# uguryagmur/RealTimeObjectDetection

Hardware: AMD Instinct MI355X
Metric: frames/sec YOLOv3 608x608 bs=8 (Darknet.forward + write_results; 2 batches in flight, write_results_async on a second stream) (higher is better)
Workload: dtype f16x2-split (3 MFMA products, f32 accumulate); 1 GPU; YOLOv3 cfg 608x608 batch=8 per GPU, split-f16 MFMA conv + fused head + GPU NMS (BASELINE configs[2]); precision=f16s3, tiles=autotune (this run), parallelism=frame-shard x1, in_flight_batches=2, detections_last_step=1699, candidates_last_step=1914, f16_range_overflow=False

## Files before the change

### realtimeobjectdetection_amd/csrc/capi.cpp

```cpp
#include <cstring>
#include <new>

#include "plan.h"

namespace rtod { const std::string& last_error_string(); }
using namespace rtod;

struct rtod_plan { Plan p; };

#define RTOD_GUARD_BEGIN try {
#define RTOD_GUARD_END                                                                   \
    } catch (const std::bad_alloc&) { set_error("out of host memory"); return RTOD_E_ARG; } \
      catch (const std::exception& e) { set_error("internal error: %s", e.what()); return RTOD_E_ARG; } \
      catch (...) { set_error("internal error"); return RTOD_E_ARG; }

extern "C" {

int rtod_version(void) { return 100; }

int rtod_last_error(char* buf, size_t len) {
    if (!buf || !len) return RTOD_E_ARG;
    const std::string& e = last_error_string();
    const size_t n = e.size() < len - 1 ? e.size() : len - 1;
    memcpy(buf, e.data(), n);
    buf[n] = 0;
    return RTOD_OK;
}

int rtod_device_count(int* out) {
    if (!out) return RTOD_E_ARG;
    int n = 0;
    hipError_t e = hipGetDeviceCount(&n);
    if (e != hipSuccess) { *out = 0; (void)hipGetLastError(); return RTOD_OK; }
    *out = n;
    return RTOD_OK;
}

static int plan_create(const char* cfg_text, size_t len, int height, int width, int max_batch, int device, rtod_plan** out) {
    rtod_plan* h = new rtod_plan();
    h->p.height = height; h->p.width = width; h->p.max_batch = max_batch; h->p.device = device;
    int rc = h->p.parse(std::string(cfg_text, len));
    if (!rc) rc = h->p.resolve_shapes();
    if (!rc) rc = h->p.plan_buffers();
    if (rc) { delete h; return rc; }
    *out = h;
    return RTOD_OK;
}

int rtod_plan_create(const char* cfg_text, size_t len, int height, int width, int max_batch, int device, rtod_plan** out) {
    RTOD_GUARD_BEGIN
    if (!cfg_text || !out) { set_error("plan_create: null pointer"); return RTOD_E_ARG; }
    *out = nullptr;
    if (height < 1 || width < 1 || max_batch < 1 || device < 0) { set_error("plan_create: bad geometry %dx%d batch %d device %d", height, width, max_batch, device); return RTOD_E_ARG; }
    if (height != width) { set_error("plan_create: only square inputs are supported (the reference derives every stride from net_info['height']); use rtod_plan_create_rect"); return RTOD_E_ARG; }
    return plan_create(cfg_text, len, height, width, max_batch, device, out);
    RTOD_GUARD_END
}

int rtod_plan_create_rect(const char* cfg_text, size_t len, int height, int width, int max_batch, int device, rtod_plan** out) {
    RTOD_GUARD_BEGIN
    if (!cfg_text || !out) { set_error("plan_create_rect: null pointer"); return RTOD_E_ARG; }
    *out = nullptr;
    if (height < 1 || width < 1 || max_batch < 1 || device < 0) { set_error("plan_create_rect: bad geometry %dx%d batch %d device %d", height, width, max_batch, device); return RTOD_E_ARG; }
    return plan_create(cfg_text, len, height, width, max_batch, device, out);
    RTOD_GUARD_END
}

int rtod_plan_destroy(rtod_plan* plan) {
    delete plan;
    return RTOD_OK;
}

int rtod_plan_get_info(const rtod_plan* plan, rtod_plan_info* o) {
    if (!plan || !o) { set_error("plan_get_info: null pointer"); return RTOD_E_ARG; }
    const Plan& p = plan->p;
    memset(o, 0, sizeof(*o));
    o->n_layers = (int32_t)p.layers.size(); o->n_launches = (int32_t)p.launches.size();
    o->height = p.height; o->width = p.width; o->max_batch = p.max_batch;
    o->total_rows = p.total_rows; o->attrs = p.attrs;
    o->n_weight_floats = p.n_weight_floats; o->conv_flops_per_frame = p.conv_flops;
    o->arena_bytes = p.arena_floats * 4; o->packed_weight_bytes = p.packed_floats * 4;
    return RTOD_OK;
}

int rtod_plan_get_launch(const rtod_plan* plan, int index, rtod_launch_info* out) {
    if (!plan || !out || index < 0 || index >= (int)plan->p.launches.size()) { set_error("plan_get_launch: bad index"); return RTOD_E_ARG; }
    plan->p.fill_launch_info(index, out, plan->p.tuned.empty() ? plan->p.max_batch : plan->p.tuned.rbegin()->first);
    return RTOD_OK;
}

int rtod_plan_describe(const rtod_plan* plan, char* buf, size_t len, size_t* needed) {
    RTOD_GUARD_BEGIN
    if (!plan) { set_error("plan_describe: null plan"); return RTOD_E_ARG; }
    const std::string s = plan->p.describe();
    if (needed) *needed = s.size() + 1;
    if (buf && len) {
        const size_t n = s.size() < len - 1 ? s.size() : len - 1;
        memcpy(buf, s.data(), n);
        buf[n] = 0;
    }
    return RTOD_OK;
    RTOD_GUARD_END
}

const char* rtod_conv_variant_name(int variant) {
    if (variant == 100 + STEM2_VARIANT) return "conv_stem2_f16s3<2 x 4x16, stem + 3x3 s2 + 1x1>";
    if (variant >= 100 + PATCH_VARIANT_BASE && variant < 100 + PATCH_VARIANT_BASE + PATCH_MODES) return conv_patch_mode_info(variant - 100 - PATCH_VARIANT_BASE).name;
    if (variant >= 100 + PWD_VARIANT_BASE && variant < 100 + PWD_VARIANT_BASE + PWD_MODES) return conv_pwd_mode_info(variant - 100 - PWD_VARIANT_BASE).name;
    if (variant >= 100 + RING_VARIANT_BASE && variant < 100 + RING_VARIANT_BASE + RING_MODES) return conv_ring_mode_info(variant - 100 - RING_VARIANT_BASE).name;
    if (variant >= 100 + BAND_VARIANT_BASE && variant < 100 + BAND_VARIANT_BASE + BAND_MODES) return conv_band_mode_info(variant - 100 - BAND_VARIANT_BASE).name;
    if (variant >= 100 && variant < 100 + HV_COUNT) return conv_f16s3_variant_info(variant - 100).name;
    if (variant < 0 || variant % 10 >= CV_COUNT || variant / 10 > 2) return "";
    static const char* const kSliced[2][CV_COUNT] = {
        {"conv_igemm_f32<128x128,w64x64,k-slices>", "conv_igemm_f32<128x64,w64x32,k-slices>", "conv_igemm_f32<64x64,w32x32,k-slices>", "conv_igemm_f32<128x32,w32x32,k-slices>"},
        {"conv_igemm_f32<128x128,w64x64,wg per k-slice>", "conv_igemm_f32<128x64,w64x32,wg per k-slice>", "conv_igemm_f32<64x64,w32x32,wg per k-slice>", "conv_igemm_f32<128x32,w32x32,wg per k-slice>"}};
    if (variant >= 10) return kSliced[variant / 10 - 1][variant % 10];
    return conv_variant_info(variant).name;
}

int rtod_conv_kernel_name(int variant, int epilogue, char* buf, size_t len) {
    if (!buf || len == 0) { set_error("conv_kernel_name: null buffer"); return RTOD_E_ARG; }
    int n = -1;
    if (variant >= 100 + PATCH_VARIANT_BASE) n = conv_patch_kernel_name(variant - 100 - PATCH_VARIANT_BASE, epilogue, buf, len);
    else if (variant >= 100 + PWD_VARIANT_BASE) n = conv_pwd_kernel_name(variant - 100 - PWD_VARIANT_BASE, epilogue, buf, len);
    else if (variant >= 100 + RING_VARIANT_BASE) n = conv_ring_kernel_name(variant - 100 - RING_VARIANT_BASE, epilogue, buf, len);
    else if (variant >= 100 + BAND_VARIANT_BASE) n = conv_band_kernel_name(variant - 100 - BAND_VARIANT_BASE, epilogue, buf, len);
    else if (variant >= 100) n = conv_f16s3_kernel_name(variant - 100, epilogue, buf, len);
    else n = conv_f32_kernel_name(variant, buf, len);
    if (n < 0 || (size_t)n >= len) { set_error("conv_kernel_name: unknown variant %d or buffer too small", variant); return RTOD_E_ARG; }
    return RTOD_OK;
}

int rtod_plan_launch_kernel_name(const rtod_plan* plan, int index, char* buf, size_t len) {
    RTOD_GUARD_BEGIN
    if (!plan || !buf || len == 0 || index < 0 || index >= (int)plan->p.launches.size()) { set_error("launch_kernel_name: bad args"); return RTOD_E_ARG; }
    rtod_launch_info li;
    plan->p.fill_launch_info(index, &li, plan->p.tuned.empty() ? plan->p.max_batch : plan->p.tuned.rbegin()->first);
    buf[0] = 0;
    if (li.kind != LK_CONV || li.flops_per_frame == 0) return RTOD_OK;
    int epi = li.fused_decode ? 2 : (li.fused_pointwise ? (li.fused_residual ? 4 : 3) : (li.fused_residual ? 1 : 0));
    if (plan->p.precision == 2 && li.variant >= 100) epi |= EPI_F16;
    int n = -1;
    if (li.variant == 100 + STEM2_VARIANT) n = conv_stem2_kernel_name(li.fused_pointwise, buf, len);
    else return rtod_conv_kernel_name(li.variant, epi, buf, len);
    if (n < 0 || (size_t)n >= len) { set_error("launch_kernel_name: buffer too small"); return RTOD_E_ARG; }
    return RTOD_OK;
    RTOD_GUARD_END
}

int rtod_plan_set_precision(rtod_plan* plan, int mode) {
    if (!plan || mode < 0 || mode > 2) { set_error("set_precision: mode must be 0 (fp32), 1 (f16 split) or 2 (plain f16)"); return RTOD_E_ARG; }
    if (plan->p.d_weights) { set_error("set_precision: must be called before rtod_plan_load_weights"); return RTOD_E_STATE; }
    if (mode >= 1) { const int rc = plan->p.check_split_supported(mode); if (rc) return rc; }
    plan->p.precision = mode;
    plan->p.layout_weights();
    return RTOD_OK;
}

int rtod_plan_set_option(rtod_plan* plan, const char* name, int value) {
    RTOD_GUARD_BEGIN
    if (!plan) { set_error("set_option: null plan"); return RTOD_E_ARG; }
    return plan->p.set_option(name, value);
    RTOD_GUARD_END
}

int rtod_plan_set_overflow_flag(rtod_plan* plan, int32_t* flag_dev) {
    if (!plan) { set_error("set_overflow_flag: null plan"); return RTOD_E_ARG; }
    plan->p.overflow_flag = flag_dev;
    return RTOD_OK;
}

int rtod_plan_load_weights(rtod_plan* plan, const float* w, size_t n_floats) {
    RTOD_GUARD_BEGIN
    if (!plan) { set_error("load_weights: null plan"); return RTOD_E_ARG; }
    return plan->p.load_weights(w, n_floats);
    RTOD_GUARD_END
}

int rtod_forward(rtod_plan* plan, const float* x_dev, int batch, float* out_dev, void* stream) {
    RTOD_GUARD_BEGIN
    if (!plan) { set_error("forward: null plan"); return RTOD_E_ARG; }
    return plan->p.forward(x_dev, batch, out_dev, (hipStream_t)stream, nullptr);
    RTOD_GUARD_END
}

int rtod_plan_autotune(rtod_plan* plan, const float* x_dev, int batch, float* out_dev, void* stream) {
    RTOD_GUARD_BEGIN
    if (!plan) { set_error("autotune: null plan"); return RTOD_E_ARG; }
    return plan->p.forward(x_dev, batch, out_dev, (hipStream_t)stream, nullptr, true);
    RTOD_GUARD_END
}

int rtod_plan_get_tiles(const rtod_plan* plan, int batch, int* variants, int capacity) {
    if (!plan) { set_error("get_tiles: null plan"); return RTOD_E_ARG; }
    auto it = plan->p.tuned.find(batch);
    if (it == plan->p.tuned.end()) { set_error("get_tiles: batch %d has no tile table (run rtod_plan_autotune first)", batch); return RTOD_E_STATE; }
    const int n = (int)it->second.size();
    if (variants) {
        if (capacity < n) { set_error("get_tiles: capacity %d < %d launches", capacity, n); return RTOD_E_ARG; }
        for (int i = 0; i < n; ++i) variants[i] = it->second[i];
    }
    return n;
}

int rtod_plan_set_tiles(rtod_plan* plan, int batch, const int* variants, int count) {
    RTOD_GUARD_BEGIN
    if (!plan) { set_error("set_tiles: null plan"); return RTOD_E_ARG; }
    return plan->p.set_tiles(batch, variants, count);
    RTOD_GUARD_END
}

int rtod_forward_timed(rtod_plan* plan, const float* x_dev, int batch, float* out_dev, void* stream, float* launch_ms) {
    RTOD_GUARD_BEGIN
    if (!plan || !launch_ms) { set_error("forward_timed: null pointer"); return RTOD_E_ARG; }
    return plan->p.forward(x_dev, batch, out_dev, (hipStream_t)stream, launch_ms);
    RTOD_GUARD_END
}

int rtod_plan_set_train_decode(rtod_plan* plan, int train) {
    if (!plan) { set_error("set_train_decode: null plan"); return RTOD_E_ARG; }
    plan->p.train_decode = train ? 1 : 0;
    return RTOD_OK;
}

int rtod_plan_set_keep_all_layers(rtod_plan* plan, int keep) {
    if (!plan) { set_error("set_keep_all_layers: null plan"); return RTOD_E_ARG; }
    if (plan->p.d_arena) { set_error("set_keep_all_layers: must be called before rtod_plan_load_weights"); return RTOD_E_STATE; }
    plan->p.keep_all = keep != 0;
    plan->p.assign_arena();
    return RTOD_OK;
}

int rtod_plan_layer_shape(const rtod_plan* plan, int layer, int* c, int* h, int* w) {
    if (!plan || layer < 0 || layer >= (int)plan->p.layers.size() || !c || !h || !w) { set_error("layer_shape: bad args"); return RTOD_E_ARG; }
    const View v = plan->p.view_of(layer);
    if (v.C == 0) { set_error("layer %d is fused into its consumer and has no materialised output", layer); return RTOD_E_STATE; }
    *c = v.C; *h = v.H; *w = v.W;
    return RTOD_OK;
}

int rtod_plan_read_layer(rtod_plan* plan, int layer, int batch, float* out_dev_nchw, void* stream) {
    RTOD_GUARD_BEGIN
    if (!plan || layer < 0 || layer >= (int)plan->p.layers.size()) { set_error("read_layer: bad args"); return RTOD_E_ARG; }
    if (batch < 1 || batch > plan->p.max_batch) { set_error("read_layer: bad batch"); return RTOD_E_ARG; }
    const View v = plan->p.view_of(layer);
    if (!v.base) { set_error("layer %d has no materialised output (fused) or weights not loaded", layer); return RTOD_E_STATE; }
    return launch_view_to_nchw(v, batch, out_dev_nchw, (hipStream_t)stream);
    RTOD_GUARD_END
}

int rtod_plan_bn_batch_stats(rtod_plan* plan, int layer, double* mean_host, double* var_host, int channels, void* stream) {
    RTOD_GUARD_BEGIN
    if (!plan || !mean_host || !var_host || layer < 0 || layer >= (int)plan->p.layers.size()) { set_error("bn_batch_stats: bad args"); return RTOD_E_ARG; }
    if (!plan->p.opt_bn_batch_stats || !plan->p.d_bn_stats) { set_error("bn_batch_stats: the plan does not run batch-statistics BatchNorm (option bn_batch_stats, weights loaded)"); return RTOD_E_STATE; }
    for (const auto& pc : plan->p.convs) {
        if (pc.layer != layer) continue;
        if (pc.stats_off < 0 || channels != plan->p.layers[layer].cout) { set_error("bn_batch_stats: layer %d has no BatchNorm / %d channels", layer, plan->p.layers[layer].cout); return RTOD_E_ARG; }
        RTOD_HIP(hipSetDevice(plan->p.device));
        RTOD_HIP(hipStreamSynchronize((hipStream_t)stream));
        RTOD_HIP(hipMemcpy(mean_host, plan->p.d_bn_stats + pc.stats_off, sizeof(double) * channels, hipMemcpyDeviceToHost));
        RTOD_HIP(hipMemcpy(var_host, plan->p.d_bn_stats + pc.stats_off + pc.Npad, sizeof(double) * channels, hipMemcpyDeviceToHost));
        return RTOD_OK;
    }
    set_error("bn_batch_stats: layer %d is not a convolution", layer);
    return RTOD_E_ARG;
    RTOD_GUARD_END
}

int rtod_plan_bn_update_running(rtod_plan* plan, int batch, float* const* running_mean_dev, float* const* running_var_dev, int n_bn,
                                double momentum, void* stream) {
    RTOD_GUARD_BEGIN
    if (!plan || !running_mean_dev || !running_var_dev || batch < 1 || batch > plan->p.max_batch) { set_error("bn_update_running: bad args"); return RTOD_E_ARG; }
    if (!plan->p.opt_bn_batch_stats || !plan->p.d_bn_stats) { set_error("bn_update_running: the plan does not run batch-statistics BatchNorm (option bn_batch_stats, weights loaded)"); return RTOD_E_STATE; }
    std::vector<BnUpdateEntry> ent;
    for (const auto& pc : plan->p.convs) {
        if (pc.stats_off < 0) continue;
        const int k = (int)ent.size();
        if (k >= n_bn) { set_error("bn_update_running: %d pointers for more BatchNorm layers", n_bn); return RTOD_E_ARG; }
        if (!running_mean_dev[k] || !running_var_dev[k]) { set_error("bn_update_running: null buffer %d", k); return RTOD_E_ARG; }
        const View v = plan->p.view_of(pc.layer);
        const auto& L = plan->p.layers[pc.layer];
        const int64_t n = (int64_t)batch * L.hout * L.wout;
        (void)v;
        ent.push_back(BnUpdateEntry{running_mean_dev[k], running_var_dev[k], pc.stats_off, (double)n / (double)(n > 1 ? n - 1 : 1), pc.Npad, L.cout});
    }
    if ((int)ent.size() != n_bn) { set_error("bn_update_running: the plan has %d BatchNorm layers, %d pointers given", (int)ent.size(), n_bn); return RTOD_E_ARG; }
    if (ent.empty()) return RTOD_OK;
    RTOD_HIP(hipSetDevice(plan->p.device));
    return launch_bn_update_running(ent.data(), (int)ent.size(), plan->p.d_bn_stats, momentum, (hipStream_t)stream);
    RTOD_GUARD_END
}

int rtod_predict_transform(const float* raw_dev, int batch, int attrs, int grid, int n_anchors, const float* anchors_wh,
                           int inp_dim, int train, float* out_dev, void* stream) {
    RTOD_GUARD_BEGIN
    if (!raw_dev || !out_dev || !anchors_wh) { set_error("predict_transform: null pointer"); return RTOD_E_ARG; }
    if (batch < 1 || attrs < 5 || grid < 1 || n_anchors < 1 || n_anchors > 4 || inp_dim < grid) { set_error("predict_transform: bad shape"); return RTOD_E_ARG; }
    const int stride = inp_dim / grid;
    if (inp_dim / stride != grid) { set_error("predict_transform: grid %d inconsistent with inp_dim %d (util.py:195 would mis-shape)", grid, inp_dim); return RTOD_E_ARG; }
    DecodeArgs d; d.enabled = 1; d.GH = grid; d.GW = grid; d.attrs = attrs; d.n_anchors = n_anchors; d.train = train ? 1 : 0; d.stride = (float)stride;
    for (int a = 0; a < n_anchors; ++a) {
        d.aw[a] = (float)((double)anchors_wh[2 * a] / (double)stride);
        d.ah[a] = (float)((double)anchors_wh[2 * a + 1] / (double)stride);
    }
    d.img_stride = (int64_t)grid * grid * n_anchors * attrs; d.head_off = 0;
    return launch_decode(raw_dev, (int64_t)n_anchors * attrs * grid * grid, (int64_t)grid * grid, grid, 1, batch, d, out_dev, (hipStream_t)stream);
    RTOD_GUARD_END
}

int rtod_confidence_mask(const float* pred_dev, int64_t rows, int attrs, float confidence, float* out_dev, void* stream) {
    return launch_confidence_mask(pred_dev, rows, attrs, confidence, out_dev, (hipStream_t)stream);
}

int rtod_bbox_iou(const float* box1_dev, const float* boxes_dev, int k, int row_stride, float* iou_dev, void* stream) {
    return launch_bbox_iou(box1_dev, boxes_dev, k, row_stride, iou_dev, (hipStream_t)stream);
}

int rtod_prep_image(const uint8_t* img_dev, int height, int width, int bgr, int inp_dim, float* out_dev, void* stream) {
    RTOD_GUARD_BEGIN
    return launch_prep_image(img_dev, height, width, bgr, inp_dim, out_dev, (hipStream_t)stream);
    RTOD_GUARD_END
}

int rtod_prep_frames(const uint8_t* frames_dev, int batch, int height, int width, int bgr, int out_h, int out_w, float* out_dev, void* stream) {
    RTOD_GUARD_BEGIN
    return launch_prep_frames(frames_dev, batch, height, width, bgr, out_h, out_w, out_dev, (hipStream_t)stream);
    RTOD_GUARD_END
}

int rtod_write_results_workspace(int batch, int n, size_t* bytes) {
    if (!bytes || batch < 1 || n < 1) { set_error("write_results_workspace: bad args"); return RTOD_E_ARG; }
    *bytes = nms_workspace_bytes(batch, n);
    return RTOD_OK;
}

int rtod_write_results(const float* pred_dev, int batch, int n, int num_class, float confidence, float nms_conf,
                       float* out_dev, int cap, int32_t* counts_dev, void* workspace_dev, size_t workspace_bytes, void* stream) {
    RTOD_GUARD_BEGIN
    return launch_write_results(pred_dev, batch, n, num_class, confidence, nms_conf, out_dev, cap, counts_dev,
                                workspace_dev, workspace_bytes, (hipStream_t)stream);
    RTOD_GUARD_END
}

int rtod_nms_class_offset(const float* pred_dev, int batch, int n, int num_class, float confidence, float iou_thr, float max_wh, int max_det,
                          float* out_dev, int cap, int32_t* counts_dev, void* workspace_dev, size_t workspace_bytes, void* stream) {
    RTOD_GUARD_BEGIN
    return launch_nms_class_offset(pred_dev, batch, n, num_class, confidence, iou_thr, max_wh, max_det, out_dev, cap, counts_dev,
                                   workspace_dev, workspace_bytes, (hipStream_t)stream);
    RTOD_GUARD_END
}

}
```

### realtimeobjectdetection_amd/csrc/conv_bandd_common.h

```cpp
#pragma once
#include "conv_f16s3_common.h"

namespace rtod {

#ifdef RTOD_TIMELINE
constexpr int BD_EPI_BLOCKS = 2048;
static __device__ unsigned long long g_bandd_epi[BD_EPI_BLOCKS * 5];
#define BD_ESTAMP(slot) { const unsigned long long tn_ = __builtin_amdgcn_s_memtime(); et_[slot] += tn_ - eprev_; eprev_ = tn_; }
#else
#define BD_ESTAMP(slot)
#endif

template <int NBASE, int PER = 2> __device__ __forceinline__ void bandd_wait_vmcnt_plus(int n) {
    static_assert(((NBASE == 4 || NBASE == 8) && PER == 2) || ((NBASE == 2 || NBASE == 4) && PER == 1), "two B sets of 1, 2 or 4 loads");
    asm volatile("" : "+s"(n));
    if (n == 0) vmcnt<NBASE>();
    else if (n == 1) vmcnt<NBASE + PER>();
    else if (n == 2) vmcnt<NBASE + 2 * PER>();
    else if (n == 3) vmcnt<NBASE + 3 * PER>();
    else if (n == 4) vmcnt<NBASE + 4 * PER>();
    else vmcnt<NBASE + 5 * PER>();
}

template <int BM, int BN, int WM, int WN, int NT, int RG, bool RES, int KG, bool F16 = false>
__device__ __forceinline__ void bandd_epilogue(const ConvArgs& a, f32x4 (&acc)[WM / 16][WN / 16], unsigned char* smem, int bm, int bn, int tid,
                                               int wm, int wn, int lr, int lh, int M, int kg) {
    constexpr int TM = WM / 16, TN = WN / 16, MT = 16, NE = 4, TS = BN;
    static_assert(BM % RG == 0 && RG % 16 == 0, "epilogue pass");
#ifdef RTOD_TIMELINE
    unsigned long long et_[5] = {0, 0, 0, 0, 0};
    unsigned long long eprev_ = __builtin_amdgcn_s_memtime();
#endif
    float* T = reinterpret_cast<float*>(smem);
    float amax = 0.f;
    const float escale = SPLIT_SCALE;
    constexpr int GPR = BN / 8;
    constexpr int NG = (RG * GPR + NT - 1) / NT;
    constexpr int NP = BM / RG;
    float bias_j[TN], inv_j[TN];
#pragma unroll
    for (int j = 0; j < TN; ++j) {
        const int n = bn * BN + wn * WN + j * MT + lr;
        const int nc = n < a.Cout ? n : 0;
        const float b = a.bias[nc], iv = a.inv_scale[nc];
        bias_j[j] = n < a.Cout ? b : 0.f; inv_j[j] = n < a.Cout ? iv : 0.f;
    }
    f16x8 rq_h[RES ? NP : 1][RES ? NG : 1], rq_l[RES ? NP : 1][RES ? NG : 1];
    static_assert(NT % GPR == 0, "epilogue items: constant row step");
    constexpr int RSTEP = NT / GPR;
    const int er = tid / GPR, ec8 = (tid - er * GPR) * 8;
    const bool ecol = bn * BN + ec8 < a.Cout;
    if constexpr (RES) {
        const _Float16* rh0 = reinterpret_cast<const _Float16*>(a.res) + a.res_coff + bn * BN;
        const int64_t rstep = (int64_t)RSTEP * 2 * a.res_ldc;
        const _Float16* const q0 = rh0 + (int64_t)(bm * BM + er) * 2 * a.res_ldc + ec8;
#pragma unroll
        for (int p = 0; p < NP; ++p) {
            const _Float16* q = q0 + (int64_t)(p * RG) * 2 * a.res_ldc;
#pragma unroll
            for (int i = 0; i < NG; ++i) {
                const int m = bm * BM + p * RG + er + i * RSTEP;
                const _Float16* qq = (er + i * RSTEP < RG && m < M && ecol) ? q : rh0;
                rq_h[p][i] = *reinterpret_cast<const f16x8*>(qq);
                if constexpr (!F16) rq_l[p][i] = *reinterpret_cast<const f16x8*>(qq + a.res_ldc);
                q += rstep;
            }
        }
    }
    __syncthreads();
    BD_ESTAMP(0)
#pragma unroll
    for (int rg = 0; rg < BM; rg += RG) {
        if constexpr (KG == 2) {
            if (kg == 1) {
#pragma unroll
                for (int i = 0; i < TM; ++i) {
                    const int r0 = wm * WM + i * MT;
                    if (r0 >= rg && r0 < rg + RG) {
#pragma unroll
                        for (int j = 0; j < TN; ++j)
#pragma unroll
                            for (int e = 0; e < NE; ++e) T[(r0 - rg + e + 4 * lh) * TS + wn * WN + j * MT + lr] = acc[i][j][e];
                    }
                }
            }
            __syncthreads();
        }
        if (KG == 1 || kg == 0) {
#pragma unroll
            for (int j = 0; j < TN; ++j) {
                const int nl = wn * WN + j * MT + lr;
                const float bias = bias_j[j] * escale, inv = inv_j[j] * escale;
                auto col = [&](auto act) {
#pragma unroll
                    for (int i = 0; i < TM; ++i) {
                        const int r0 = wm * WM + i * MT;
                        if (r0 >= rg && r0 < rg + RG) {
#pragma unroll
                            for (int e = 0; e < NE; ++e) {
                                const int rl = r0 - rg + e + 4 * lh;
                                float s = acc[i][j][e];
                                if constexpr (KG == 2) s += T[rl * TS + nl];
                                float v = s * inv + bias;
                                if constexpr (decltype(act)::value == 2) v = silu_scaled(v, 1.0f / escale);
                                else if constexpr (decltype(act)::value == 1) v = __builtin_fmaxf(v, v * 0.1f);
                                T[rl * TS + nl] = v;
                            }
                        }
                    }
                };
                if (a.leaky == 2) col(std::integral_constant<int, 2>{});
                else if (a.leaky) col(std::integral_constant<int, 1>{});
                else col(std::integral_constant<int, 0>{});
            }
        }
        BD_ESTAMP(1)
        __syncthreads();
        BD_ESTAMP(2)
        _Float16* oq = reinterpret_cast<_Float16*>(a.out) + a.out_coff + bn * BN + (int64_t)(bm * BM + rg + er) * 2 * a.out_ldc + ec8;
        const int64_t ostep = (int64_t)RSTEP * 2 * a.out_ldc;
#pragma unroll
        for (int gi = 0; gi < NG; ++gi, oq += ostep) {
            const int r = er + gi * RSTEP;
            const int m = bm * BM + rg + r;
            if (r >= RG || m >= M || !ecol) continue;
            const f32x4 v0 = *reinterpret_cast<const f32x4*>(T + r * TS + ec8);
            const f32x4 v1 = *reinterpret_cast<const f32x4*>(T + r * TS + ec8 + 4);
            float v[8] = {v0[0], v0[1], v0[2], v0[3], v1[0], v1[1], v1[2], v1[3]};
            if constexpr (RES && F16) {
                const f16x8 qh = rq_h[rg / RG][gi];
#pragma unroll
                for (int e = 0; e < 8; ++e) v[e] += (float)qh[e];
            } else if constexpr (RES) {
                const f16x8 qh = rq_h[rg / RG][gi], ql = rq_l[rg / RG][gi];
#pragma unroll
                for (int e = 0; e < 8; ++e) v[e] += (float)qh[e] + (float)ql[e];
            }
            if constexpr (F16) {
                f16x8 ph;
#pragma unroll
                for (int e = 0; e < 8; ++e) ph[e] = f16_sat(v[e], amax);
                store_act16(oq, ph, false);
            } else {
                f16x8 ph, pl;
#pragma unroll
                for (int e = 0; e < 8; ++e) { _Float16 h, l; split_f16(v[e], h, l, amax); ph[e] = h; pl[e] = l; }
                store_act16(oq, ph, false);
                store_act16(oq + a.out_ldc, pl, false);
            }
        }
        BD_ESTAMP(3)
        if (rg + RG < BM) __syncthreads();
        BD_ESTAMP(4)
    }
#ifdef RTOD_TIMELINE
    if (threadIdx.x == 0 && blockIdx.x < BD_EPI_BLOCKS) for (int i = 0; i < 5; ++i) g_bandd_epi[blockIdx.x * 5 + i] = et_[i];
#endif
    split_overflow_report(a.ovf, amax);
}

}
```

### realtimeobjectdetection_amd/csrc/conv_pwd_f16s3.hip

```cpp
#include "conv_bandd_common.h"

namespace rtod {

template <int BM, int NW, int NST, int MINW, int EPI>
__global__ __launch_bounds__(NW * 64, MINW)
void conv_pwd_f16s3_kernel(const ConvArgs a, const int grid_m, const int grid_n) {
    constexpr bool F16 = epi_f16(EPI);
    constexpr int LB = F16 ? 2 : 4, LP = F16 ? 1 : 2;
    constexpr int BN = NW * 32, NT = NW * 64, TM = BM / 16, TN = 2;
    constexpr int SLAB = BM * 256;
    constexpr int NP = BM / 8;
    constexpr int NPP = (NP + NW - 1) / NW;
    static_assert(BM % 16 == 0 && NPP >= 1 && NPP <= 8, "slab pieces per wave");
    static_assert(NST >= 2 && NST <= 4, "ring depth");
    constexpr int RG = BM * BN * 4 <= 32768 ? BM : (BM / 2) * BN * 4 <= 32768 ? BM / 2 : BM / 4;
    constexpr int WAIT_B = 2 * LB + LP * NPP;
    constexpr int WAIT_SLAB = 2 * LB + (NST - 2) * (LP * NPP + 2 * LB);
    constexpr int WAIT_SLAB_PRO = 2 * LB + (NST - 2) * LP * NPP;

    extern __shared__ __attribute__((aligned(16))) unsigned char smem[];
    const int nwg = grid_m * grid_n;
    int bid = blockIdx.x;
    if (!a.xcd_by_n) bid = xcd_remap(bid, nwg);
    const int bm = bid / grid_n, bn = bid - bm * grid_n;
    const int tid = (int)threadIdx.x;
    const int wave = __builtin_amdgcn_readfirstlane(tid >> 6), lane = tid & 63;
    const int lr = lane & 15, lh = lane >> 4;
    const int M = a.B * a.Hi * a.Wi;
    const int m0 = bm * BM;
    const unsigned PS = (unsigned)a.in_ldc * 4u;
    const unsigned lo_plane = (unsigned)a.in_ldc * 2u;

    const __amdgpu_buffer_rsrc_t rs_a = buffer_rsrc(a.in, a.in_bytes);
    const __amdgpu_buffer_rsrc_t rs_wh = buffer_rsrc(a.w_hi, a.w_bytes);
    const __amdgpu_buffer_rsrc_t rs_wl = buffer_rsrc(a.w_lo, a.w_bytes);
    const unsigned lds0 = (unsigned)(size_t)smem;
    const int NS = a.Cin / 64;

    unsigned dma_vo[NPP];
#pragma unroll
    for (int k = 0; k < NPP; ++k) {
        const int p = wave + k * NW;
        const int r = lane >> 3;
        const int m = m0 + p * 8 + r;
        dma_vo[k] = (p < NP && m < M) ? (unsigned)m * PS + (unsigned)(a.in_coff + (((lane & 7) ^ r) << 3)) * 2u : OOB;
    }
    auto dma_slab = [&](int js) __attribute__((always_inline)) {
        const bool live = js < NS;
        const unsigned soff = (unsigned)js * 128u;
        const unsigned base = lds0 + (unsigned)((js % NST) * SLAB);
#pragma unroll
        for (int k = 0; k < NPP; ++k) {
            const int p = wave + k * NW;
            const unsigned dst = p < NP ? base + (unsigned)((p >> 1) * 4096 + (p & 1) * 1024) : lds0 + (unsigned)(NST * SLAB);
            if constexpr (F16) lds_dma(rs_a, live ? dma_vo[k] : OOB, soff, dst);
            else lds_dma_pair<0x800>(rs_a, live ? dma_vo[k] : OOB, soff, lo_plane + soff, dst);
        }
    };
    const int wn = wave;
    const int n0 = bn * BN + wn * 32;
    const unsigned bvoff = n0 + lr < a.Npad ? (unsigned)((n0 + lr) * 32 + lh * 8) * 2u : OOB;
    const unsigned wchunk = (unsigned)a.Npad * (HBK * 2);
    const int nsteps = 2 * NS;
    u32x4 Bq[4][TN][2];
    auto load_b = [&](int t, u32x4 (&q)[TN][2]) __attribute__((always_inline)) {
        const unsigned vo = t < nsteps ? bvoff : OOB;
        const unsigned koff = (unsigned)t * wchunk;
        q[0][0] = buffer_load_b128(rs_wh, vo, koff);
        if constexpr (!F16) q[0][1] = buffer_load_b128(rs_wl, vo, koff);
        q[1][0] = buffer_load_b128<1024>(rs_wh, vo, koff);
        if constexpr (!F16) q[1][1] = buffer_load_b128<1024>(rs_wl, vo, koff);
    };

    f32x4 acc[TM][TN];
#pragma unroll
    for (int i = 0; i < TM; ++i)
#pragma unroll
        for (int j = 0; j < TN; ++j)
#pragma unroll
            for (int e = 0; e < 4; ++e) acc[i][j][e] = 0.f;

    typedef const f16x8 __attribute__((address_space(3))) lds_f16x8;
    const int rbase = (lr >> 3) * 1024 + (lr & 7) * 128;
    int xq0 = rbase + ((lh ^ (lr & 7)) << 4);
    int xq1 = rbase + (((4 + lh) ^ (lr & 7)) << 4);
    f16x8 Ah[3], Al[3];
    auto read_unit = [&](int q, int i, int slotoff, f16x8& h, f16x8& l) __attribute__((always_inline)) {
        const int o = (q ? xq1 : xq0) + slotoff;
        h = *reinterpret_cast<lds_f16x8*>((unsigned)(o + 4096 * i));
        if constexpr (!F16) l = *reinterpret_cast<lds_f16x8*>((unsigned)(o + 4096 * i + 2048));
    };

#pragma unroll
    for (int s = 0; s < NST - 1; ++s) dma_slab(s);
    load_b(0, Bq[0]);
    load_b(1, Bq[1]);

    __builtin_amdgcn_s_setprio(2);
    auto slab_body = [&](int j, auto par_c) __attribute__((always_inline)) {
        constexpr int par = decltype(par_c)::value;
        asm volatile("" : "+v"(xq0), "+v"(xq1));
        if (j < NST - 1) vmcnt<WAIT_SLAB_PRO>(); else vmcnt<WAIT_SLAB>();
        __builtin_amdgcn_sched_barrier(0);
        __builtin_amdgcn_s_barrier();
        dma_slab(j + NST - 1);
        const int slotoff = (int)lds0 + (j % NST) * SLAB;
        read_unit(0, 0, slotoff, Ah[0], Al[0]);
        read_unit(1 / TM, 1 % TM, slotoff, Ah[1], Al[1]);
        __builtin_amdgcn_sched_barrier(0);
#pragma unroll
        for (int u = 0; u < 2 * TM; ++u) {
            const int q = u / TM, i = u % TM;
            if (i == 0) {
                if (q == 0) load_b(2 * j + 2, Bq[(2 * par + 2) % 4]); else load_b(2 * j + 3, Bq[(2 * par + 3) % 4]);
                vmcnt<WAIT_B>();
                if (q == 0) tie_bset<F16>(Bq[2 * par]); else tie_bset<F16>(Bq[2 * par + 1]);
                __builtin_amdgcn_sched_barrier(0);
            }
            if (u + 2 < 2 * TM) read_unit((u + 2) / TM, (u + 2) % TM, slotoff, Ah[(u + 2) % 3], Al[(u + 2) % 3]);
            const f16x8 ah = Ah[u % 3], al = Al[u % 3];
#pragma unroll
            for (int jn = 0; jn < TN; ++jn) {
                const f16x8 bh = __builtin_bit_cast(f16x8, Bq[2 * par + q][jn][0]);
                if constexpr (F16) { acc[i][jn] = __builtin_amdgcn_mfma_f32_16x16x32_f16(ah, bh, acc[i][jn], 0, 0, 0); continue; }
                const f16x8 bl = __builtin_bit_cast(f16x8, Bq[2 * par + q][jn][1]);
                acc[i][jn] = __builtin_amdgcn_mfma_f32_16x16x32_f16(al, bh, acc[i][jn], 0, 0, 0);
                acc[i][jn] = __builtin_amdgcn_mfma_f32_16x16x32_f16(ah, bl, acc[i][jn], 0, 0, 0);
                acc[i][jn] = __builtin_amdgcn_mfma_f32_16x16x32_f16(ah, bh, acc[i][jn], 0, 0, 0);
            }
            __builtin_amdgcn_sched_barrier(0);
        }
    };
#pragma unroll 1
    for (int j = 0; j < NS; j += 2) {
        slab_body(j, std::integral_constant<int, 0>{});
        if (j + 1 < NS) slab_body(j + 1, std::integral_constant<int, 1>{});
    }
    vmcnt<0>();
    tie_bset<F16>(Bq[0]); tie_bset<F16>(Bq[1]); tie_bset<F16>(Bq[2]); tie_bset<F16>(Bq[3]);
    __builtin_amdgcn_sched_barrier(0);
    __builtin_amdgcn_s_setprio(0);

    bandd_epilogue<BM, BN, BM, 32, NT, RG, epi_kind(EPI) == EPI_SPLIT_RES, 1, F16>(a, acc, smem, bm, bn, tid, 0, wn, lr, lh, M, 0);
}

template <int BM, int NW, int NST, int MINW>
static int launch_pwd(const ConvArgs& a, hipStream_t s) {
    constexpr int BN = NW * 32, NT = NW * 64;
    constexpr int RG = BM * BN * 4 <= 32768 ? BM : (BM / 2) * BN * 4 <= 32768 ? BM / 2 : BM / 4;
    const int M = a.B * a.Ho * a.Wo;
    const int gm = (M + BM - 1) / BM, gn = (a.Cout + BN - 1) / BN;
    ConvArgs ax = a;
    ax.xcd_by_n = (gn % 8 == 0 && (int64_t)a.Cout * a.K > (int64_t)M * a.Cin) ? 1 : 0;
    constexpr int ring_bytes = NST * BM * 256 + ((BM / 8) % NW ? 4096 : 0), epi_bytes = RG * BN * 4;
    constexpr int lds = ring_bytes > epi_bytes ? ring_bytes : epi_bytes;
    static_assert(lds <= 160 * 1024, "LDS");
    const int fe = a.f16 ? 1 : 0;
    auto k_res = fe ? conv_pwd_f16s3_kernel<BM, NW, NST, MINW, EPI_SPLIT_RES | EPI_F16> : conv_pwd_f16s3_kernel<BM, NW, NST, MINW, EPI_SPLIT_RES>;
    auto k_plain = fe ? conv_pwd_f16s3_kernel<BM, NW, NST, MINW, EPI_SPLIT | EPI_F16> : conv_pwd_f16s3_kernel<BM, NW, NST, MINW, EPI_SPLIT>;
    if constexpr (lds > 64 * 1024) {
        static std::atomic<unsigned long long> attr_done[2] = {{0}, {0}};
        if (int rc = lds_opt_in(attr_done[fe], lds, "conv_pwd_f16s3", k_res, k_plain)) return rc;
    }
    if (a.res) hipLaunchKernelGGL(k_res, dim3(gm * gn), dim3(NT), lds, s, ax, gm, gn);
    else hipLaunchKernelGGL(k_plain, dim3(gm * gn), dim3(NT), lds, s, ax, gm, gn);
    return hip_fail(hipGetLastError(), "conv_pwd_f16s3 launch");
}

#define RTOD_PWD_TILES(X) \
    X(0, 64, 4, 3, 3) X(1, 32, 4, 3, 3) X(2, 128, 4, 3, 1) X(3, 64, 8, 3, 1) X(4, 64, 4, 2, 3) X(5, 32, 4, 4, 3) X(6, 96, 4, 2, 3) X(7, 96, 4, 3, 2) X(8, 48, 4, 3, 3) X(9, 48, 4, 4, 3) X(10, 64, 2, 2, 4)

#define RTOD_X_INFO(idx, bm, nw, nst, minw) {bm, nw * 32, "conv_pwd_f16s3<" #bm "x" #nw "w,r" #nst ">"},
static const ConvVariantInfo kPwdModes[PWD_MODES] = { RTOD_PWD_TILES(RTOD_X_INFO) };
#undef RTOD_X_INFO
const ConvVariantInfo& conv_pwd_mode_info(int idx) { return kPwdModes[idx < 0 || idx >= PWD_MODES ? 0 : idx]; }

bool conv_pwd_supported(int ksize, int stride, int pad, int cin) { return ksize == 1 && stride == 1 && pad == 0 && cin >= 64 && cin % 64 == 0; }

int conv_pwd_kernel_name(int idx, int epi, char* buf, size_t len) {
#define RTOD_X_NAME(i, bm, nw, nst, minw) \
    if (idx == i) return snprintf(buf, len, "void rtod::conv_pwd_f16s3_kernel<" #bm ", " #nw ", " #nst ", " #minw ", %d>(rtod::ConvArgs, int, int)", epi);
    RTOD_PWD_TILES(RTOD_X_NAME)
#undef RTOD_X_NAME
    return -1;
}

int launch_conv_pwd_f16s3(const ConvArgs& a, int idx, hipStream_t s) {
    if (int rc = check_split_conv_args(a, "launch_conv_pwd", true)) return rc;
    if (!conv_pwd_supported(a.kh, a.stride, a.pad, a.Cin) || a.kw != 1 || a.Ho != a.Hi || a.Wo != a.Wi || a.dec.enabled || a.pw_wh) {
        set_error("launch_conv_pwd: unsupported shape (k=%d s=%d pad=%d Cin=%d)", a.kh, a.stride, a.pad, a.Cin); return RTOD_E_ARG;
    }
    if (a.in_ldc % 8 || a.in_coff % 8 || a.K != a.Kpad || a.K != a.Cin || a.Npad % 128) { set_error("launch_conv_pwd: bad view / K"); return RTOD_E_ARG; }
    switch (idx) {
#define RTOD_X_CASE(i, bm, nw, nst, minw) case i: return launch_pwd<bm, nw, nst, minw>(a, s);
        RTOD_PWD_TILES(RTOD_X_CASE)
#undef RTOD_X_CASE
    }
    set_error("launch_conv_pwd: mode %d unsupported", idx);
    return RTOD_E_ARG;
}

}
```

### realtimeobjectdetection_amd/csrc/plan.cpp

```cpp
#include "plan.h"

#include <algorithm>
#include <cctype>
#include <cmath>
#include <cstdarg>
#include <cstdlib>
#include <cstring>
#include <map>
#include <mutex>
#include <sstream>

namespace rtod {

static thread_local std::string g_err;

void set_error(const char* fmt, ...) {
    char buf[1024];
    va_list ap;
    va_start(ap, fmt);
    vsnprintf(buf, sizeof(buf), fmt, ap);
    va_end(ap);
    g_err = buf;
}
const std::string& last_error_string() { return g_err; }

int hip_fail(hipError_t e, const char* what) {
    if (e == hipSuccess) return RTOD_OK;
    set_error("HIP error %d (%s) at %s", (int)e, hipGetErrorString(e), what);
    return RTOD_E_HIP;
}

const char* layer_type_name(int t) {
    static const char* n[] = {"convolutional", "shortcut", "route", "upsample", "maxpool", "yolo"};
    return (t >= 0 && t < 6) ? n[t] : "?";
}

Plan::~Plan() {
    for (auto e : events) (void)hipEventDestroy(e);
    if (d_arena) (void)hipFree(d_arena);
    if (d_scratch) (void)hipFree(d_scratch);
    if (d_bn_stats) (void)hipFree(d_bn_stats);
    if (d_bn_partial) (void)hipFree(d_bn_partial);
    if (d_weights) (void)hipFree(d_weights);
}

static std::string rstrip(const std::string& s) {
    size_t e = s.size();
    while (e > 0 && isspace((unsigned char)s[e - 1])) --e;
    return s.substr(0, e);
}
static std::string lstrip(const std::string& s) {
    size_t b = 0;
    while (b < s.size() && isspace((unsigned char)s[b])) ++b;
    return s.substr(b);
}

static bool to_int(const std::string& s, int& out) {
    const std::string t = rstrip(lstrip(s));
    if (t.empty()) return false;
    char* end = nullptr;
    long v = strtol(t.c_str(), &end, 10);
    if (*end) return false;
    out = (int)v;
    return true;
}

static std::vector<std::string> split(const std::string& s, char d) {
    std::vector<std::string> out;
    std::string cur;
    for (char c : s) {
        if (c == d) { out.push_back(cur); cur.clear(); } else cur.push_back(c);
    }
    out.push_back(cur);
    return out;
}

struct Block { std::string type; std::map<std::string, std::string> kv; };

static int parse_blocks(const std::string& text, std::vector<Block>& blocks) {
    Block cur;
    bool have = false;
    for (const std::string& raw : split(text, '\n')) {
        if (raw.empty()) continue;
        if (raw[0] == '#') continue;
        const std::string line = rstrip(lstrip(raw));
        if (line.empty()) continue;
        if (line[0] == '[') {
            if (have) blocks.push_back(cur);
            cur = Block();
            have = true;
            cur.type = rstrip(line.substr(1, line.size() >= 2 ? line.size() - 2 : 0));
        } else {
            const auto parts = split(line, '=');
            if (parts.size() != 2 || !have) { set_error("cfg: malformed line '%s'", line.c_str()); return RTOD_E_CFG; }
            cur.kv[rstrip(parts[0])] = lstrip(parts[1]);
        }
    }
    if (have) blocks.push_back(cur);
    if (blocks.empty() || blocks[0].type != "net") { set_error("cfg: first block must be [net]"); return RTOD_E_CFG; }
    return RTOD_OK;
}

#define CFG_INT(blk, key, var)                                                                  \
    do {                                                                                        \
        auto _it = (blk).kv.find(key);                                                          \
        if (_it == (blk).kv.end() || !to_int(_it->second, var)) {                               \
            set_error("cfg: layer %d [%s]: missing/invalid '%s'", i, (blk).type.c_str(), key);  \
            return RTOD_E_CFG;                                                                  \
        }                                                                                       \
    } while (0)

int Plan::parse(const std::string& text) {
    std::vector<Block> blocks;
    int rc = parse_blocks(text, blocks);
    if (rc) return rc;
    net_info = blocks[0].kv;
    layers.clear();
    for (size_t bi = 1; bi < blocks.size(); ++bi) {
        const Block& b = blocks[bi];
        const int i = (int)bi - 1;
        Layer L;
        L.index = i;
        if (b.type == "convolutional") {
            L.type = LT_CONV;
            int bn = 0;
            auto it = b.kv.find("batch_normalize");
            L.bn = (it != b.kv.end() && to_int(it->second, bn) && bn != 0);
            int padflag = 0;
            CFG_INT(b, "filters", L.cout);
            CFG_INT(b, "size", L.size);
            CFG_INT(b, "stride", L.stride);
            CFG_INT(b, "pad", padflag);
            L.pad = padflag ? (L.size - 1) / 2 : 0;
            auto act = b.kv.find("activation");
            if (act == b.kv.end()) { set_error("cfg: layer %d: missing activation", i); return RTOD_E_CFG; }
            L.leaky = act->second == "leaky";
            L.act = L.leaky ? 1 : (act->second == "silu" || act->second == "swish") ? 2 : 0;
            if (L.cout < 1 || L.size < 1 || L.stride < 1) { set_error("cfg: layer %d: bad conv geometry", i); return RTOD_E_CFG; }
        } else if (b.type == "upsample") {
            L.type = LT_UPSAMPLE;
            int st = 0;
            CFG_INT(b, "stride", st);
            L.stride = 2;
            auto md = b.kv.find("mode");
            L.nearest = md != b.kv.end() && md->second == "nearest";
        } else if (b.type == "maxpool") {
            L.type = LT_MAXPOOL;
            CFG_INT(b, "size", L.size);
            CFG_INT(b, "stride", L.stride);
            int sym = 0;
            auto sy = b.kv.find("symmetric");
            if (sy != b.kv.end() && to_int(sy->second, sym) && sym) L.pool_pad = (L.size - 1) / 2;
            if (L.size < 1 || L.stride < 1) { set_error("cfg: layer %d: bad pool geometry", i); return RTOD_E_CFG; }
        } else if (b.type == "shortcut") {
            L.type = LT_SHORTCUT;
            int from = 0;
            CFG_INT(b, "from", from);
            L.srcs = {i - 1, i + from};
        } else if (b.type == "route") {
            L.type = LT_ROUTE;
            auto it = b.kv.find("layers");
            if (it == b.kv.end()) { set_error("cfg: layer %d: route without layers", i); return RTOD_E_CFG; }
            for (const std::string& tok : split(it->second, ',')) {
                int v = 0;
                if (!to_int(tok, v)) { set_error("cfg: layer %d: bad route entry '%s'", i, tok.c_str()); return RTOD_E_CFG; }
                L.srcs.push_back(v > 0 ? v : i + v);
            }
            if (L.srcs.empty() || L.srcs.size() > 4) {
                set_error("cfg: layer %d: route with %zu sources unsupported", i, L.srcs.size()); return RTOD_E_CFG;
            }
        } else if (b.type == "yolo") {
            L.type = LT_YOLO;
            auto m = b.kv.find("mask"), a = b.kv.find("anchors");
            if (m == b.kv.end() || a == b.kv.end()) { set_error("cfg: layer %d: yolo without mask/anchors", i); return RTOD_E_CFG; }
            std::vector<int> av;
            for (const std::string& tok : split(a->second, ',')) { int v; if (!to_int(tok, v)) { set_error("cfg: bad anchor"); return RTOD_E_CFG; } av.push_back(v); }
            for (const std::string& tok : split(m->second, ',')) {
                int v;
                if (!to_int(tok, v) || v < 0 || 2 * v + 1 >= (int)av.size()) { set_error("cfg: layer %d: bad mask", i); return RTOD_E_CFG; }
                L.anchors.push_back({av[2 * v], av[2 * v + 1]});
            }
            CFG_INT(b, "classes", L.classes);
            auto dv = b.kv.find("decode");
            L.decode_v5 = dv != b.kv.end() && dv->second == "v5";
            if (L.anchors.empty() || L.anchors.size() > 4) { set_error("cfg: layer %d: 1..4 anchors per head supported", i); return RTOD_E_CFG; }
        } else {
            set_error("Unknown block error: A unknown block is provided: [%s]", b.type.c_str());
            return RTOD_E_CFG;
        }
        layers.push_back(L);
    }
    if (layers.empty()) { set_error("cfg: no layers"); return RTOD_E_CFG; }
    return RTOD_OK;
}

int Plan::resolve_shapes() {
    int pc = 3, ph = height, pw = width;
    int row_off = 0;
    int64_t woff = 0;
    conv_flops = 0;
    attrs = 0;
    bool prev_is_decoded = false;
    for (auto& L : layers) {
        const int i = L.index;
        auto src_ok = [&](int s) { return s >= 0 && s < i; };
        if ((L.type == LT_CONV || L.type == LT_UPSAMPLE || L.type == LT_MAXPOOL || L.type == LT_YOLO) && prev_is_decoded) {
            set_error("cfg: layer %d consumes a decoded yolo tensor (unsupported)", i); return RTOD_E_CFG;
        }
        L.cin = pc; L.hin = ph; L.win = pw;
        switch (L.type) {
            case LT_CONV:
                L.hout = (ph + 2 * L.pad - L.size) / L.stride + 1;
                L.wout = (pw + 2 * L.pad - L.size) / L.stride + 1;
                if (L.hout < 1 || L.wout < 1) { set_error("cfg: layer %d: empty conv output", i); return RTOD_E_CFG; }
                L.w_off = woff;
                woff += (L.bn ? 4 : 1) * (int64_t)L.cout + (int64_t)L.cout * L.cin * L.size * L.size;
                conv_flops += 2ll * L.hout * L.wout * L.cout * L.cin * L.size * L.size;
                break;
            case LT_UPSAMPLE: L.cout = pc; L.hout = 2 * ph; L.wout = 2 * pw; break;
            case LT_MAXPOOL:
                L.cout = pc;
                if (L.pool_pad) { L.hout = (ph + 2 * L.pool_pad - L.size) / L.stride + 1; L.wout = (pw + 2 * L.pool_pad - L.size) / L.stride + 1; }
                else if (L.stride != 1) { L.hout = (ph - L.size) / L.stride + 1; L.wout = (pw - L.size) / L.stride + 1; }
                else { L.hout = ph; L.wout = pw; }
                if (L.hout < 1 || L.wout < 1) { set_error("cfg: layer %d: empty pool output", i); return RTOD_E_CFG; }
                break;
            case LT_SHORTCUT: {
                if (i < 1 || !src_ok(L.srcs[1])) { set_error("cfg: layer %d: shortcut source out of range", i); return RTOD_E_CFG; }
                const Layer& a = layers[L.srcs[0]]; const Layer& b = layers[L.srcs[1]];
                if (a.cout != b.cout || a.hout != b.hout || a.wout != b.wout) { set_error("cfg: layer %d: shortcut shape mismatch", i); return RTOD_E_CFG; }
                L.cout = a.cout; L.hout = a.hout; L.wout = a.wout;
                break;
            }
            case LT_ROUTE: {
                int c = 0;
                for (int s : L.srcs) {
                    if (!src_ok(s)) { set_error("cfg: layer %d: route source %d out of range", i, s); return RTOD_E_CFG; }
                    if (layers[s].hout != layers[L.srcs[0]].hout || layers[s].wout != layers[L.srcs[0]].wout) { set_error("cfg: layer %d: route spatial mismatch", i); return RTOD_E_CFG; }
                    c += layers[s].cout;
                }
                L.cout = c; L.cin = c; L.hout = layers[L.srcs[0]].hout; L.wout = layers[L.srcs[0]].wout;
                break;
            }
            case LT_YOLO: {
                if (i < 1) { set_error("cfg: yolo as first layer"); return RTOD_E_CFG; }
                const int A = (int)L.anchors.size();
                if (pc != A * (5 + L.classes)) { set_error("cfg: layer %d: head has %d channels, expected %d", i, pc, A * (5 + L.classes)); return RTOD_E_CFG; }
                if (ph > height || pw > width || height / (height / ph) != ph || width / (width / pw) != pw) {
                    set_error("cfg: layer %d: grid %dx%d does not divide input %dx%d", i, ph, pw, height, width); return RTOD_E_CFG;
                }
                if (height / ph != width / pw) {
                    set_error("cfg: layer %d: head grid %dx%d has stride %d along y but %d along x for input %dx%d (one integer stride on both axes is required)",
                              i, ph, pw, height / ph, width / pw, height, width);
                    return RTOD_E_CFG;
                }
                if (attrs && attrs != 5 + L.classes) { set_error("cfg: heads with different class counts"); return RTOD_E_CFG; }
                attrs = 5 + L.classes;
                L.cout = pc; L.hout = ph; L.wout = pw;
                L.row_offset = row_off; L.rows = ph * pw * A;
                row_off += L.rows;
                break;
            }
        }
        if (L.type == LT_YOLO) {
            prev_is_decoded = true;
            pc = layers[i - 1].cout; ph = layers[i - 1].hout; pw = layers[i - 1].wout;
        } else {
            prev_is_decoded = false;
            pc = L.cout; ph = L.hout; pw = L.wout;
        }
        if (L.type == LT_ROUTE || L.type == LT_SHORTCUT) prev_is_decoded = false;
    }
    total_rows = row_off;
    n_weight_floats = woff;
    if (total_rows == 0) { set_error("cfg: no yolo layer (the reference would return [])"); return RTOD_E_CFG; }
    return RTOD_OK;
}

static int resolve_alias(const std::vector<Layer>& layers, int i) {
    while (layers[i].alias_of >= 0) i = layers[i].alias_of;
    return i;
}

void Plan::reset_planning() {
    for (auto& L : layers) { L.fused_into = -1; L.fused_away = false; L.buf = -1; L.coff = 0; L.alias_of = -1; }
    bufs.clear(); launches.clear(); convs.clear(); input_buf = -1;
    tuned.clear(); tune_cache.clear(); tuning.clear();
}

int Plan::set_option(const char* name, int value) {
    if (!name) { set_error("set_option: null name"); return RTOD_E_ARG; }
    if (d_weights) { set_error("set_option: must be called before rtod_plan_load_weights"); return RTOD_E_STATE; }
    const std::string k(name);
    bool* flag = nullptr; int* num = nullptr;
    if (k == "fuse_pointwise") flag = &opt_fuse_pointwise;
    else if (k == "ring_kernel") flag = &opt_ring_kernel;
    else if (k == "pwd_kernel") flag = &opt_pwd_kernel;
    else if (k == "stem2_kernel") flag = &opt_stem2_kernel;
    else if (k == "k_slices") flag = &opt_k_slices;
    else if (k == "bn_batch_stats") {
        if (value && height != width) { set_error("set_option: bn_batch_stats is not supported on a rectangular plan (%dx%d)", height, width); return RTOD_E_ARG; }
        flag = &opt_bn_batch_stats;
    }
    else if (k == "k_slice_workgroups") flag = &opt_k_slice_workgroups;
    else if (k == "patch_kernel") flag = &opt_patch_kernel;
    else if (k == "stem_kernel") flag = &opt_stem_kernel;
    else if (k == "band_kernel") flag = &opt_band_kernel;
    else if (k == "fuse_shortcut") flag = &opt_fuse_shortcut;
    else if (k == "fuse_decode") flag = &opt_fuse_decode;
    else if (k == "zero_copy_concat") flag = &opt_zero_copy_concat;
    else if (k == "force_f16s3_variant") num = &opt_force_f16s3_variant;
    else if (k == "force_f32_variant") num = &opt_force_f32_variant;
    else { set_error("set_option: unknown option '%s'", name); return RTOD_E_ARG; }
    const bool old_flag = flag ? *flag : false; const int old_num = num ? *num : 0;
    if (flag) *flag = value != 0; else *num = value;
    reset_planning();
    int rc = plan_buffers();
    if (!rc && precision >= 1) rc = check_split_supported(precision);
    if (rc) {
        const std::string msg = last_error_string();
        if (flag) *flag = old_flag; else *num = old_num;
        reset_planning();
        (void)plan_buffers();
        set_error("%s", msg.c_str());
    }
    return rc;
}

int Plan::plan_buffers() {
    const int n = (int)layers.size();
    std::vector<std::vector<int>> cons(n);
    for (const auto& L : layers) {
        const int i = L.index;
        switch (L.type) {
            case LT_CONV: case LT_UPSAMPLE: case LT_MAXPOOL: case LT_YOLO: if (i > 0) cons[i - 1].push_back(i); break;
            case LT_SHORTCUT: case LT_ROUTE: for (int s : L.srcs) cons[s].push_back(i); break;
        }
    }
    for (auto& L : layers) {
        if (L.type == LT_ROUTE && L.srcs.size() == 1) L.alias_of = L.srcs[0];
        if (L.type == LT_YOLO) L.alias_of = L.index - 1;
    }
    for (auto& L : layers) {
        const int i = L.index;
        if (i == 0) continue;
        Layer& P = layers[i - 1];
        if (P.type != LT_CONV || P.fused_into >= 0 || cons[i - 1].size() != 1) continue;
        if (L.type == LT_SHORTCUT && L.srcs[1] != i - 1 && opt_fuse_shortcut) { P.fused_into = i; L.fused_away = true; }
        else if (L.type == LT_YOLO && cons[i].empty() && opt_fuse_decode) { P.fused_into = i; L.fused_away = true; }
    }
    auto materialised = [&](const Layer& L) {
        if (L.alias_of >= 0) return false;
        if (L.type == LT_CONV && L.fused_into >= 0) return false;
        if (L.type == LT_ROUTE) return true;
        return true;
    };
    bufs.clear();
    std::vector<int> placed_buf(n, -1), placed_off(n, 0);
    std::vector<std::vector<std::pair<int, int>>> route_copy(n);
    for (auto& L : layers) {
        if (L.type != LT_ROUTE || L.srcs.size() < 2) continue;
        Buffer b; b.C = L.cout; b.H = L.hout; b.W = L.wout;
        const int bid = (int)bufs.size();
        bufs.push_back(b);
        L.buf = bid; L.coff = 0;
        int off = 0;
        for (int s : L.srcs) {
            const int p = resolve_alias(layers, s);
            const Layer& PL = layers[p];
            const bool can = opt_zero_copy_concat && materialised(PL) && PL.type != LT_ROUTE && placed_buf[p] < 0 && off % 4 == 0 && PL.cout % 4 == 0 &&
                             std::count(L.srcs.begin(), L.srcs.end(), s) == 1;
            if (can) { placed_buf[p] = bid; placed_off[p] = off; }
            else route_copy[L.index].push_back({s, off});
            off += layers[s].cout;
        }
    }
    for (auto& L : layers) {
        if (!materialised(L) || L.buf >= 0) continue;
        if (L.type == LT_YOLO) continue;
        if (placed_buf[L.index] >= 0) { L.buf = placed_buf[L.index]; L.coff = placed_off[L.index]; continue; }
        Buffer b; b.C = L.cout; b.H = L.hout; b.W = L.wout;
        if (b.C % 4) { set_error("layer %d: %d channels not a multiple of 4 (unsupported for an intermediate tensor)", L.index, b.C); return RTOD_E_CFG; }
        L.buf = (int)bufs.size(); L.coff = 0;
        bufs.push_back(b);
    }
    {
        Buffer b; b.C = 4; b.H = height; b.W = width;
        input_buf = (int)bufs.size();
        bufs.push_back(b);
    }
    launches.clear();
    convs.clear();
    if (layers[0].type != LT_CONV) { set_error("cfg: first layer must be convolutional"); return RTOD_E_CFG; }
    const bool use_stem = layers[0].size == 3 && layers[0].pad == 1 && layers[0].cin == 3 && layers[0].cout % 32 == 0 &&
                          layers[0].cout <= 64 && layers[0].fused_into < 0 && opt_stem_kernel && !(opt_bn_batch_stats && layers[0].bn);
    if (!use_stem) { Launch l; l.kind = LK_PACK; l.layer = 0; launches.push_back(l); }
    for (auto& L : layers) {
        const int i = L.index;
        Launch l; l.layer = i;
        switch (L.type) {
            case LT_CONV: {
                l.kind = LK_CONV; l.in_layer = i - 1; l.out_layer = i;
                if (L.fused_into >= 0) {
                    const Layer& F = layers[L.fused_into];
                    if (F.type == LT_SHORTCUT) { l.out_layer = F.index; l.in2_layer = F.srcs[1]; }
                    else {
                        l.out_layer = -2;
                        DecodeArgs d; d.enabled = 1; d.GH = F.hout; d.GW = F.wout; d.attrs = 5 + F.classes; d.n_anchors = (int)F.anchors.size();
                        const int stride = height / F.hout;
                        d.stride = (float)stride;
                        for (size_t a = 0; a < F.anchors.size(); ++a) {
                            d.aw[a] = (float)((double)F.anchors[a].first / (double)stride);
                            d.ah[a] = (float)((double)F.anchors[a].second / (double)stride);
                            if (F.decode_v5) { d.aw[a] = (float)F.anchors[a].first; d.ah[a] = (float)F.anchors[a].second; }
                        }
                        d.v5 = F.decode_v5 ? 1 : 0;
                        d.img_stride = (int64_t)total_rows * attrs; d.head_off = (int64_t)F.row_offset * attrs;
                        l.dec = d;
                    }
                }
                PackedConv pc; pc.layer = i; pc.cin_p = (i == 0) ? 4 : L.cin;
                if (i == 0 && use_stem) { pc.stem = true; l.kind = LK_STEM; }
                if (pc.cin_p % 4) { set_error("layer %d: %d input channels not a multiple of 4", i, pc.cin_p); return RTOD_E_CFG; }
                pc.K = L.size * L.size * pc.cin_p; pc.Kpad = (pc.K + 31) / 32 * 32; pc.Npad = (L.cout + 127) / 128 * 128;
                l.conv_slot = (int)convs.size();
                convs.push_back(pc);
                launches.push_back(l);
                break;
            }
            case LT_UPSAMPLE: l.kind = LK_UPSAMPLE; l.in_layer = i - 1; l.out_layer = i; launches.push_back(l); break;
            case LT_MAXPOOL: l.kind = LK_MAXPOOL; l.in_layer = i - 1; l.out_layer = i; launches.push_back(l); break;
            case LT_SHORTCUT:
                if (!L.fused_away) { l.kind = LK_ADD; l.in_layer = L.srcs[0]; l.in2_layer = L.srcs[1]; l.out_layer = i; launches.push_back(l); }
                break;
            case LT_ROUTE:
                for (auto& sc : route_copy[i]) { Launch c; c.kind = LK_COPY; c.layer = i; c.in_layer = sc.first; c.out_buf = L.buf; c.out_coff = sc.second; c.out_layer = i; launches.push_back(c); }
                break;
            case LT_YOLO:
                if (!L.fused_away) {
                    l.kind = LK_DECODE; l.in_layer = i - 1; l.out_layer = -2;
                    DecodeArgs d; d.enabled = 1; d.GH = L.hout; d.GW = L.wout; d.attrs = 5 + L.classes; d.n_anchors = (int)L.anchors.size();
                    const int stride = height / L.hout;
                    d.stride = (float)stride;
                    for (size_t a = 0; a < L.anchors.size(); ++a) {
                        d.aw[a] = (float)((double)L.anchors[a].first / (double)stride);
                        d.ah[a] = (float)((double)L.anchors[a].second / (double)stride);
                        if (L.decode_v5) { d.aw[a] = (float)L.anchors[a].first; d.ah[a] = (float)L.anchors[a].second; }
                    }
                    d.v5 = L.decode_v5 ? 1 : 0;
                    d.img_stride = (int64_t)total_rows * attrs; d.head_off = (int64_t)L.row_offset * attrs;
                    l.dec = d;
                    launches.push_back(l);
                }
                break;
        }
    }
    for (size_t i = 0; i + 1 < launches.size(); ++i) {
        Launch& h = launches[i]; Launch& g = launches[i + 1];
        if (h.kind != LK_CONV || g.kind != LK_CONV || h.out_layer < 0 || g.out_layer < 0 || g.in2_layer >= 0 || h.pw_host >= 0) continue;
        const Layer& H = layers[h.layer]; const Layer& G = layers[g.layer];
        if (g.in_layer != h.out_layer || G.size != 1 || G.stride != 1 || G.pad != 0 || G.cin != H.cout) continue;
        if (H.cout % 32 || H.cout > 64 || (G.cout != 16 && G.cout != 32 && G.cout != 64) || G.fused_into >= 0) continue;
        if (conv_band_supported(H.size, H.stride, H.pad, H.cin, H.win) && H.hout == H.hin) continue;
        h.pw_guest = (int)i + 1; g.pw_host = (int)i;
    }
    stem2_pattern = false;
    if (launches.size() >= 2 && launches[0].kind == LK_STEM && launches[1].kind == LK_CONV && launches[1].layer == 1 && launches[1].in_layer == 0 &&
        launches[1].in2_layer < 0 && launches[1].out_layer == 1 && cons[0].size() == 1 && n > 1) {
        const Layer& L0 = layers[0]; const Layer& L1 = layers[1];
        int pwc = 0;
        if (launches[1].pw_guest >= 0) pwc = layers[launches[launches[1].pw_guest].layer].cout;
        stem2_pattern = L0.bn && L1.bn && L0.act <= 1 && L1.act <= 1 && (launches[1].pw_guest < 0 || layers[launches[launches[1].pw_guest].layer].act <= 1) && conv_stem2_supported(L0.size, L0.stride, L0.pad, L0.cin, L0.cout, L1.size, L1.stride, L1.pad, L1.cout, pwc) &&
                        (pwc == 0 || pwc == 32);
    }
    const int NB = (int)bufs.size();
    for (auto& b : bufs) { b.first = 1 << 30; b.last = -1; }
    auto touch = [&](int buf, int t) { if (buf < 0) return; bufs[buf].first = std::min(bufs[buf].first, t); bufs[buf].last = std::max(bufs[buf].last, t); };
    auto buf_of_layer = [&](int layer) { if (layer < 0) return input_buf; return layers[resolve_alias(layers, layer)].buf; };
    for (const auto& l : launches) {
        const int t = l.layer;
        if (l.kind == LK_PACK) { touch(input_buf, 0); continue; }
        if (l.kind == LK_STEM) { touch(buf_of_layer(l.out_layer), t); continue; }
        touch(buf_of_layer(l.in_layer), t);
        if (l.in2_layer >= 0) touch(buf_of_layer(l.in2_layer), t);
        if (l.kind == LK_COPY) touch(l.out_buf, t);
        else if (l.out_layer >= 0) touch(buf_of_layer(l.out_layer), t);
        if (l.pw_guest >= 0) touch(buf_of_layer(launches[l.pw_guest].out_layer), t);
    }
    for (int b = 0; b < NB; ++b) {
        if (bufs[b].last < 0) { bufs[b].first = bufs[b].last = 0; }
        bufs[b].floats_per_frame = (int64_t)bufs[b].C * bufs[b].H * bufs[b].W;
    }
    assign_arena();
    layout_weights();
    return RTOD_OK;
}

bool Plan::uses_split(const Layer& L, int cin_p) const {
    return precision >= 1 && L.index > 0;
}

int Plan::check_split_supported(int mode) const {
    const char* pn = mode == 2 ? "f16" : "f16s3";
    if (opt_bn_batch_stats) { set_error("precision %s unsupported with bn_batch_stats (batch-statistics BatchNorm runs on the exact-fp32 kernels)", pn); return RTOD_E_CFG; }
    for (const auto& l : launches) {
        if (l.kind == LK_ADD || l.kind == LK_COPY || l.kind == LK_DECODE) {
            set_error("precision %s unsupported for this cfg (layer %d needs a stand-alone %s kernel); use fp32", pn, l.layer,
                      l.kind == LK_ADD ? "add" : l.kind == LK_COPY ? "copy" : "decode");
            return RTOD_E_CFG;
        }
        if (l.kind == LK_CONV && l.layer > 0) {
            const Layer& L = layers[l.layer];
            if (L.cin % 32 || L.cout % 8 * (l.out_layer != -2)) {
                set_error("precision %s unsupported for this cfg (layer %d: Cin=%d Cout=%d); use fp32", pn, l.layer, L.cin, L.cout);
                return RTOD_E_CFG;
            }
        }
    }
    for (const auto& b : bufs) if (b.C % 8 && &b != &bufs[input_buf]) { set_error("precision %s: a buffer has %d channels (not a multiple of 8)", pn, b.C); return RTOD_E_CFG; }
    return RTOD_OK;
}

void Plan::layout_weights() {
    packed_floats = 0;
    bn_stats_doubles = 0;
    for (auto& pc : convs) {
        pc.stats_off = -1;
        if (opt_bn_batch_stats && layers[pc.layer].bn) { pc.stats_off = bn_stats_doubles; bn_stats_doubles += 2 * (int64_t)pc.Npad; }
    }
    for (auto& pc : convs) {
        const Layer& L = layers[pc.layer];
        pc.split = uses_split(L, pc.cin_p);
        const int64_t panel = (int64_t)pc.Npad * pc.Kpad;
        if (pc.stem && precision >= 1) {
            pc.split = true;
            pc.w_off = packed_floats; packed_floats += 16 * (int64_t)L.cout;
            pc.wl_off = packed_floats; packed_floats += 16 * (int64_t)L.cout;
            pc.s_off = packed_floats; packed_floats += L.cout;
        } else if (pc.stem) {
            pc.w_off = packed_floats; packed_floats += 28 * (int64_t)L.cout;
        } else if (pc.split) {
            pc.w_off = packed_floats; packed_floats += panel / 2;
            pc.wl_off = packed_floats; packed_floats += panel / 2;
            pc.s_off = packed_floats; packed_floats += pc.Npad;
            pc.band = conv_band_supported(L.size, L.stride, L.pad, L.cin, L.win) && L.hout == L.hin &&
                      !(L.fused_into >= 0 && layers[L.fused_into].type == LT_YOLO) && opt_band_kernel;
        } else {
            pc.w_off = packed_floats; packed_floats += panel;
            const int nkc = pc.Kpad / 32;
            pc.slice_chunks = (!opt_k_slices || L.hout * L.wout > 2704 || nkc < 8) ? 0 : nkc >= 32 ? 9 : nkc >= 16 ? 4 : 2;
        }
        pc.b_off = packed_floats; packed_floats += pc.Npad;
        if (opt_bn_batch_stats && L.bn) { pc.bn_off = packed_floats; packed_floats += 2 * (int64_t)pc.Npad; }
        packed_floats = (packed_floats + 63) / 64 * 64;
    }
}

void Plan::assign_arena() {
    const int NB = (int)bufs.size();
    std::vector<int> order(NB);
    for (int i = 0; i < NB; ++i) order[i] = i;
    std::sort(order.begin(), order.end(), [&](int a, int b) { return bufs[a].first != bufs[b].first ? bufs[a].first < bufs[b].first : a < b; });
    std::vector<int> done;
    arena_floats = 0;
    for (int id : order) {
        Buffer& B = bufs[id];
        const int64_t size = (B.floats_per_frame * max_batch + 63) / 64 * 64;
        std::vector<std::pair<int64_t, int64_t>> busy;
        for (int o : done) {
            const Buffer& O = bufs[o];
            if (!keep_all && (O.last < B.first || O.first > B.last)) continue;
            busy.push_back({O.offset, O.offset + (O.floats_per_frame * max_batch + 63) / 64 * 64});
        }
        std::sort(busy.begin(), busy.end());
        int64_t off = 0;
        for (auto& iv : busy) { if (off + size <= iv.first) break; off = std::max(off, iv.second); }
        B.offset = off;
        arena_floats = std::max(arena_floats, off + size);
        done.push_back(id);
    }
}

View Plan::view_of(int layer) const {
    View v;
    if (layer < 0) {
        const Buffer& b = bufs[input_buf];
        v.base = d_arena ? d_arena + b.offset : nullptr; v.ldc = 4; v.coff = 0; v.C = 4; v.H = height; v.W = width;
        return v;
    }
    const Layer& L = layers[resolve_alias(layers, layer)];
    if (L.buf < 0) return v;
    const Buffer& b = bufs[L.buf];
    v.split = precision;
    v.base = d_arena ? d_arena + b.offset : nullptr;
    v.ldc = b.C; v.coff = L.coff; v.C = L.cout; v.H = L.hout; v.W = L.wout;
    return v;
}

static uint16_t f32_to_f16_rn(float f) {
    uint32_t x; memcpy(&x, &f, 4);
    const uint32_t sign = (x >> 16) & 0x8000u;
    x &= 0x7FFFFFFFu;
    if (x >= 0x7F800000u) return (uint16_t)(sign | (x > 0x7F800000u ? 0x7E00u : 0x7C00u));
    if (x >= 0x477FF000u) return (uint16_t)(sign | 0x7C00u);
    if (x < 0x33000001u) return (uint16_t)sign;
    int e = (int)(x >> 23) - 127;
    uint32_t m = (x & 0x7FFFFFu) | 0x800000u;
    int shift = (e < -14) ? (13 + (-14 - e)) : 13;
    uint32_t half_m = m >> shift;
    const uint32_t rem = m & ((1u << shift) - 1), halfway = 1u << (shift - 1);
    if (rem > halfway || (rem == halfway && (half_m & 1))) ++half_m;
    uint32_t out;
    if (e < -14) out = half_m;
    else out = ((uint32_t)(e + 15) << 10) + (half_m - 0x400u);
    return (uint16_t)(sign | out);
}
static float f16_to_f32(uint16_t h) {
    const uint32_t sign = (uint32_t)(h & 0x8000u) << 16;
    const int e = (h >> 10) & 0x1F; const uint32_t m = h & 0x3FFu;
    float v;
    if (e == 0) v = std::ldexp((float)m, -24);
    else if (e == 31) v = m ? NAN : INFINITY;
    else v = std::ldexp((float)(m | 0x400u), e - 25);
    uint32_t x; memcpy(&x, &v, 4); x |= sign; memcpy(&v, &x, 4);
    return v;
}

int Plan::load_weights(const float* w, size_t n) {
    if (!w) { set_error("load_weights: null pointer"); return RTOD_E_ARG; }
    if ((int64_t)n < n_weight_floats) {
        set_error("load_weights: stream has %zu floats, network needs %lld", n, (long long)n_weight_floats);
        return RTOD_E_SIZE;
    }
    RTOD_HIP(hipSetDevice(device));
    std::vector<float> packed((size_t)packed_floats, 0.0f);
    for (const auto& pc : convs) {
        const Layer& L = layers[pc.layer];
        const float* p = w + L.w_off;
        const int C = L.cout, cin = L.cin, k = L.size;
        std::vector<double> scale(C, 1.0);
        float* bias = packed.data() + pc.b_off;
        if (L.bn && opt_bn_batch_stats) {
            float* bnp = packed.data() + pc.bn_off;
            for (int o = 0; o < C; ++o) { bias[o] = 0.f; bnp[o] = p[o]; bnp[pc.Npad + o] = p[C + o]; }
            p += 4 * C;
        } else if (L.bn) {
            const float *beta = p, *gamma = p + C, *mean = p + 2 * C, *var = p + 3 * C;
            for (int o = 0; o < C; ++o) {
                const double s = (double)gamma[o] / std::sqrt((double)var[o] + 1e-5);
                scale[o] = s;
                bias[o] = (float)((double)beta[o] - (double)mean[o] * s);
            }
            p += 4 * C;
        } else {
            for (int o = 0; o < C; ++o) bias[o] = p[o];
            p += C;
        }
        if (pc.stem && pc.split) {
            uint16_t* wh = reinterpret_cast<uint16_t*>(packed.data() + pc.w_off);
            uint16_t* wl = reinterpret_cast<uint16_t*>(packed.data() + pc.wl_off);
            float* inv = packed.data() + pc.s_off;
            const int64_t per_o = (int64_t)cin * k * k;
            for (int o = 0; o < C; ++o) {
                double mx = 0.0;
                for (int64_t q = 0; q < per_o; ++q) mx = std::max(mx, std::fabs((double)p[o * per_o + q] * scale[o]));
                int e = 0;
                if (mx > 0.0) { int ex; std::frexp(mx, &ex); e = 13 - ex; }
                e = std::max(-24, std::min(40, e));
                const double ps = std::ldexp(1.0, e);
                inv[o] = (float)(std::ldexp(1.0, -e) / (double)ACT_SCALE_F16S3);
                for (int q = 0; q < 32; ++q) { wh[o * 32 + q] = 0; wl[o * 32 + q] = 0; }
                for (int c = 0; c < cin; ++c)
                    for (int ky = 0; ky < k; ++ky)
                        for (int kx = 0; kx < k; ++kx) {
                            const float v = (float)((double)p[(((int64_t)o * cin + c) * k + ky) * k + kx] * scale[o]);
                            const float vs = (float)((double)v * ps);
                            const uint16_t h = f32_to_f16_rn(vs);
                            const int idx = o * 32 + (ky * k + kx) * 3 + c;
                            wh[idx] = h; wl[idx] = f32_to_f16_rn(vs - f16_to_f32(h));
                        }
            }
        } else if (pc.stem) {
            float* wp = packed.data() + pc.w_off;
            for (int o = 0; o < C; ++o)
                for (int c = 0; c < cin; ++c)
                    for (int ky = 0; ky < k; ++ky)
                        for (int kx = 0; kx < k; ++kx) {
                            const float v = p[(((int64_t)o * cin + c) * k + ky) * k + kx];
                            wp[(int64_t)((ky * k + kx) * 3 + c) * C + o] = (float)((double)v * scale[o]);
                        }
        } else if (!pc.split) {
            float* wp = packed.data() + pc.w_off;
            for (int o = 0; o < C; ++o)
                for (int c = 0; c < cin; ++c)
                    for (int ky = 0; ky < k; ++ky)
                        for (int kx = 0; kx < k; ++kx) {
                            const float v = p[(((int64_t)o * cin + c) * k + ky) * k + kx];
                            wp[(int64_t)o * pc.Kpad + (ky * k + kx) * pc.cin_p + c] = (float)((double)v * scale[o]);
                        }
        } else {
            uint16_t* wh = reinterpret_cast<uint16_t*>(packed.data() + pc.w_off);
            uint16_t* wl = reinterpret_cast<uint16_t*>(packed.data() + pc.wl_off);
            float* inv = packed.data() + pc.s_off;
            for (int o = 0; o < pc.Npad; ++o) inv[o] = 1.0f / ACT_SCALE_F16S3;
            const int64_t per_o = (int64_t)cin * k * k;
            for (int o = 0; o < C; ++o) {
                double mx = 0.0;
                for (int64_t q = 0; q < per_o; ++q) mx = std::max(mx, std::fabs((double)p[o * per_o + q] * scale[o]));
                int e = 0;
                if (mx > 0.0) { int ex; std::frexp(mx, &ex); e = 13 - ex; }
                e = std::max(-24, std::min(40, e));
                const double ps = std::ldexp(1.0, e);
                inv[o] = (float)(std::ldexp(1.0, -e) / (double)ACT_SCALE_F16S3);
                for (int c = 0; c < cin; ++c)
                    for (int ky = 0; ky < k; ++ky)
                        for (int kx = 0; kx < k; ++kx) {
                            const float v = (float)((double)p[(((int64_t)o * cin + c) * k + ky) * k + kx] * scale[o]);
                            const float vs = (float)((double)v * ps);
                            const uint16_t h = f32_to_f16_rn(vs);
                            const uint16_t l = f32_to_f16_rn(vs - f16_to_f32(h));
                            const int64_t idx = ((int64_t)((c / 32) * k * k + (ky * k + kx)) * pc.Npad + o) * 32 + (c % 32);
                            wh[idx] = h; wl[idx] = l;
                        }
            }
        }
    }
    if (!d_weights) RTOD_HIP(hipMalloc((void**)&d_weights, sizeof(float) * (size_t)packed_floats));
    if (!d_arena) {
        RTOD_HIP(hipMalloc((void**)&d_arena, sizeof(float) * (size_t)arena_floats));
        if (precision == 2) RTOD_HIP(hipMemsetD16((hipDeviceptr_t)d_arena, 0x7E00, 2 * (size_t)arena_floats));
        else RTOD_HIP(hipMemset(d_arena, 0, sizeof(float) * (size_t)arena_floats));
    }
    if (opt_bn_batch_stats && !d_bn_stats && bn_stats_doubles > 0) {
        RTOD_HIP(hipMalloc((void**)&d_bn_stats, sizeof(double) * (size_t)bn_stats_doubles));
        RTOD_HIP(hipMemset(d_bn_stats, 0, sizeof(double) * (size_t)bn_stats_doubles));
        int maxn = 0;
        for (const auto& pc : convs) if (pc.stats_off >= 0) maxn = std::max(maxn, pc.Npad);
        bn_partial_count = (int64_t)bn_partial_doubles(maxn);
        RTOD_HIP(hipMalloc((void**)&d_bn_partial, sizeof(double) * (size_t)bn_partial_count));
    }
    if (!d_scratch) {
        bool any = false;
        for (const auto& pc : convs) any = any || (!pc.split && !pc.stem && pc.slice_chunks > 0);
        if (any) {
            scratch_floats = 8ll << 20;
            RTOD_HIP(hipMalloc((void**)&d_scratch, sizeof(float) * (size_t)scratch_floats));
        }
    }
    RTOD_HIP(hipMemcpy(d_weights, packed.data(), sizeof(float) * (size_t)packed_floats, hipMemcpyHostToDevice));
    RTOD_HIP(hipDeviceSynchronize());
    weights_loaded = true;
    return RTOD_OK;
}

int Plan::choose_variant(const Layer& L, int batch) const {
    if (opt_force_f32_variant >= 0 && opt_force_f32_variant < CV_COUNT) return opt_force_f32_variant;
    if (L.cout <= 32) return CV_128x32;
    if (L.cout <= 64) return CV_128x64;
    const int64_t M = (int64_t)batch * L.hout * L.wout;
    const int64_t big = ((M + 127) / 128) * ((L.cout + 127) / 128);
    return big >= 512 ? CV_128x128 : CV_64x64;
}

int Plan::f32_slice_mode(const Launch& l, int batch, int variant) const {
    const PackedConv& pc = convs[l.conv_slot];
    if (pc.split || pc.stem || pc.slice_chunks <= 0) return 0;
    const Layer& L = layers[l.layer];
    const ConvVariantInfo& vi = conv_variant_info(variant);
    const int64_t M = (int64_t)batch * L.hout * L.wout;
    const int64_t tiles = ((M + vi.bm - 1) / vi.bm) * ((L.cout + vi.bn - 1) / vi.bn);
    const int64_t S = (pc.Kpad / 32 + pc.slice_chunks - 1) / pc.slice_chunks;
    return (opt_k_slice_workgroups && d_scratch && tiles < 512 && S * M * pc.Npad <= scratch_floats) ? 2 : 1;
}

static bool variant_has_f16(int v) {
    return (v >= 0 && v < HV_COUNT) || (v >= BAND_VARIANT_BASE + BAND_LDS_MODES && v < BAND_VARIANT_BASE + BAND_MODES) ||
           (v >= PWD_VARIANT_BASE && v < PWD_VARIANT_BASE + PWD_MODES);
}
static bool band_mode_ok(int precision, int mode, const Layer& L) {
    return conv_band_mode_valid(mode, L.cin, L.hin, L.win) && (precision != 2 || mode >= BAND_LDS_MODES);
}
static int band_default_mode(int precision, const Layer& L) {
    if (precision != 2) return conv_band_default_mode(L.cin, L.hin, L.win);
    for (int m = BAND_LDS_MODES; m < BAND_MODES; ++m) if (conv_band_mode_valid(m, L.cin, L.hin, L.win)) return m;
    return BAND_LDS_MODES;
}

int Plan::launch_split_variant(ConvArgs& a, const PackedConv& pc, int v, hipStream_t s) const {
    if (precision == 2 && !variant_has_f16(v)) { set_error("variant %d has no plain-f16 instance", v); return RTOD_E_STATE; }
    if (v >= PATCH_VARIANT_BASE) {
        if (pc.band) { set_error("patch variant requested for a band layer"); return RTOD_E_STATE; }
        return launch_conv_patch_f16s3(a, v - PATCH_VARIANT_BASE, s);
    }
    if (v >= PWD_VARIANT_BASE) {
        if (pc.band) { set_error("pointwise variant requested for a band layer"); return RTOD_E_STATE; }
        return launch_conv_pwd_f16s3(a, v - PWD_VARIANT_BASE, s);
    }
    if (v >= RING_VARIANT_BASE) {
        if (pc.band) { set_error("ring variant requested for a band layer"); return RTOD_E_STATE; }
        return launch_conv_ring_f16s3(a, v - RING_VARIANT_BASE, s);
    }
    if (v >= BAND_VARIANT_BASE) {
        if (v == BAND_VARIANT_BASE + BANDD_WIDE_MODE && !pc.band) return launch_conv_bandd_f16s3(a, v - BAND_VARIANT_BASE - BAND_LDS_MODES, s);
        if (!pc.band) { set_error("band variant requested for a layer without band weights"); return RTOD_E_STATE; }
        return launch_conv_band_f16s3(a, v - BAND_VARIANT_BASE, s);
    }
    return launch_conv_f16s3(a, v, s);
}

int Plan::build_conv_args(const Launch& l, int batch, float* out, ConvArgs& a) const {
    const Layer& L = layers[l.layer];
    const PackedConv& pc = convs[l.conv_slot];
    const View in = view_of(l.in_layer);
    a.in = in.base; a.in_ldc = in.ldc; a.in_coff = in.coff;
    a.B = batch; a.Hi = L.hin; a.Wi = L.win; a.Cin = pc.cin_p;
    a.w = d_weights + pc.w_off; a.bias = d_weights + pc.b_off; a.K = pc.K; a.Kpad = pc.Kpad; a.Npad = pc.Npad;
    a.in_bytes = (unsigned)std::min<int64_t>((int64_t)batch * in.H * in.W * in.ldc * 4, 0xFFFFFFFFll);
    a.w_bytes = (unsigned)std::min<int64_t>((int64_t)pc.Npad * pc.Kpad * 2, 0xFFFFFFFFll);
    if (pc.split) {
        a.w_hi = reinterpret_cast<const _Float16*>(d_weights + pc.w_off);
        a.w_lo = reinterpret_cast<const _Float16*>(d_weights + pc.wl_off);
        a.inv_scale = d_weights + pc.s_off;
        a.f16 = precision == 2 ? 1 : 0;
    }
    a.kh = a.kw = L.size; a.stride = L.stride; a.pad = L.pad;
    a.Ho = L.hout; a.Wo = L.wout; a.Cout = L.cout; a.leaky = L.act;
    a.ovf = overflow_flag;
    if (in.C != pc.cin_p || in.H != L.hin || in.W != L.win) { set_error("forward: layer %d input view mismatch", l.layer); return RTOD_E_STATE; }
    if (l.out_layer == -2) { a.out = out; a.dec = l.dec; a.dec.train = train_decode; }
    else {
        const View o = view_of(l.out_layer);
        if (!o.base || o.C != L.cout || o.H != L.hout || o.W != L.wout) { set_error("forward: layer %d output view mismatch", l.layer); return RTOD_E_STATE; }
        a.out = o.base; a.out_ldc = o.ldc; a.out_coff = o.coff; a.out_split = o.split;
    }
    if (l.in2_layer >= 0) {
        const View r = view_of(l.in2_layer);
        if (!r.base || r.C != L.cout || r.H != L.hout || r.W != L.wout) { set_error("forward: layer %d residual view mismatch", l.layer); return RTOD_E_STATE; }
        a.res = r.base; a.res_ldc = r.ldc; a.res_coff = r.coff;
    }
    if (l.pw_guest >= 0 && pw_active()) {
        const Launch& g = launches[l.pw_guest];
        const Layer& G = layers[g.layer];
        const PackedConv& gc = convs[g.conv_slot];
        const View o = view_of(g.out_layer);
        if (!gc.split || gc.Kpad != L.cout || !o.base || !o.split || o.C != G.cout || o.H != L.hout || o.W != L.wout) { set_error("forward: layer %d fused pointwise mismatch", g.layer); return RTOD_E_STATE; }
        a.pw_wh = reinterpret_cast<const _Float16*>(d_weights + gc.w_off);
        a.pw_wl = reinterpret_cast<const _Float16*>(d_weights + gc.wl_off);
        a.pw_inv_scale = d_weights + gc.s_off; a.pw_bias = d_weights + gc.b_off;
        a.pw_out = o.base; a.pw_out_ldc = o.ldc; a.pw_out_coff = o.coff;
        a.pw_cout = G.cout; a.pw_k = L.cout; a.pw_leaky = G.act; a.pw_npad = gc.Npad;
    }
    return RTOD_OK;
}

static std::mutex g_tune_mutex;
static std::map<std::vector<int>, int> g_tune_memo;

int Plan::tune_launch(size_t li, ConvArgs& a, int batch, hipStream_t s) {
    const Launch& l = launches[li];
    const Layer& L = layers[l.layer];
    const bool pw = a.pw_wh != nullptr;
    const std::vector<int> key = {L.cin, L.cout, L.size, L.stride, L.hout, L.wout, l.in2_layer >= 0, l.out_layer == -2, pw ? a.pw_cout : 0,
                                  convs[l.conv_slot].band ? 1 : 0, opt_ring_kernel ? 1 : 0, opt_patch_kernel ? 1 : 0, opt_pwd_kernel ? 1 : 0, L.act,
                                  precision, L.hin, L.win, L.pad};
    auto it = tune_cache.find(key);
    if (it != tune_cache.end()) { tuning[li] = it->second; return RTOD_OK; }
    std::vector<int> gkey = key; gkey.push_back(device); gkey.push_back(batch);
    {
        std::lock_guard<std::mutex> lock(g_tune_mutex);
        auto git = g_tune_memo.find(gkey);
        if (git != g_tune_memo.end()) { tuning[li] = git->second; tune_cache[key] = git->second; return RTOD_OK; }
    }
    hipEvent_t e0, e1;
    RTOD_HIP(hipEventCreate(&e0)); RTOD_HIP(hipEventCreate(&e1));
    std::vector<int> cand;
    if (convs[l.conv_slot].band) {
        for (int m = 0; m < BAND_MODES; ++m) if (band_mode_ok(precision, m, L)) cand.push_back(BAND_VARIANT_BASE + m);
    } else {
        for (int v = 0; v < HV_COUNT; ++v) {
            const ConvVariantInfo& vi = conv_f16s3_variant_info(v);
            if (vi.bn > 2 * ((L.cout + 63) / 64 * 64) && vi.bn > 64) continue;
            if (pw && vi.bn < L.cout) continue;
            cand.push_back(v);
        }
        if (precision == 1 && !pw && L.act <= 1 && opt_patch_kernel && conv_patch_supported(L.size, L.stride, L.pad, L.cin, L.cout) && L.hout == L.hin && l.out_layer != -2)
            for (int m = 0; m < PATCH_MODES; ++m) {
                if (conv_patch_mode_info(m).bn > L.cout && conv_patch_mode_info(m).bn > 64) continue;
                if (!conv_patch_mode_valid(m, L.cin, L.cout)) continue;
                cand.push_back(PATCH_VARIANT_BASE + m);
            }
        if (bandd_wide_candidate(l, L)) cand.push_back(BAND_VARIANT_BASE + BANDD_WIDE_MODE);
        if (pwd_candidate(l, L))
            for (int m = 0; m < PWD_MODES; ++m) {
                if (conv_pwd_mode_info(m).bn > 128 && conv_pwd_mode_info(m).bn > (L.cout + 127) / 128 * 128) continue;
                cand.push_back(PWD_VARIANT_BASE + m);
            }
        if (precision == 1 && !pw && L.act <= 1 && opt_ring_kernel)
            for (int m = 0; m < RING_MODES; ++m) {
                const ConvVariantInfo& vi = conv_ring_mode_info(m);
                if (vi.bn > 2 * ((L.cout + 63) / 64 * 64) && vi.bn > 64) continue;
                cand.push_back(RING_VARIANT_BASE + m);
            }
    }
    int best_v = variant_for(l, batch);
    int rc = RTOD_OK;
    auto time_variant = [&](int v, int reps, int per, float& out_ms) -> int {
        out_ms = 1e30f;
        for (int rep = 0; rep < reps; ++rep) {
            (void)hipEventRecord(e0, s);
            for (int r = 0; r < per; ++r) { const int q = launch_split_variant(a, convs[l.conv_slot], v, s); if (q) return q; }
            (void)hipEventRecord(e1, s);
            if (hipEventSynchronize(e1) != hipSuccess) return hip_fail(hipGetLastError(), "autotune sync");
            float ms = 0.f; (void)hipEventElapsedTime(&ms, e0, e1);
            out_ms = std::min(out_ms, ms / per);
        }
        return RTOD_OK;
    };
    std::vector<std::pair<float, int>> ranked;
    for (int v : cand) {
        rc = launch_split_variant(a, convs[l.conv_slot], v, s);
        if (rc) break;
        float ms; rc = time_variant(v, 3, 2, ms);
        if (rc) break;
        ranked.push_back({ms, v});
    }
    if (!rc && !ranked.empty()) {
        std::sort(ranked.begin(), ranked.end());
        const size_t top = std::min<size_t>(3, ranked.size());
        std::vector<float> fin(top, 1e30f);
        for (int round = 0; round < 5 && !rc; ++round)
            for (size_t t = 0; t < top && !rc; ++t) {
                float ms; rc = time_variant(ranked[t].second, 2, 4, ms);
                fin[t] = std::min(fin[t], ms);
            }
        if (!rc) best_v = ranked[std::min_element(fin.begin(), fin.end()) - fin.begin()].second;
    }
    (void)hipEventDestroy(e0); (void)hipEventDestroy(e1);
    if (rc) return rc;
    tuning[li] = best_v;
    tune_cache[key] = best_v;
    { std::lock_guard<std::mutex> lock(g_tune_mutex); g_tune_memo[gkey] = best_v; }
    return RTOD_OK;
}

int Plan::set_tiles(int batch, const int* variants, int count) {
    if (!variants || count != (int)launches.size() || batch <= 0 || batch > max_batch) { set_error("set_tiles: %d entries for %d launches, batch %d", count, (int)launches.size(), batch); return RTOD_E_ARG; }
    if (precision < 1) { set_error("set_tiles: split-f16 / f16 plans only"); return RTOD_E_STATE; }
    for (int i = 0; i < count; ++i) {
        const int v = variants[i];
        const Launch& l = launches[i];
        if (v < 0) continue;
        if (l.kind != LK_CONV || l.conv_slot < 0 || !convs[l.conv_slot].split) { set_error("set_tiles: launch %d is not a split-f16 convolution", i); return RTOD_E_ARG; }
        const Layer& L = layers[l.layer];
        const bool band = convs[l.conv_slot].band, hosts_pw = l.pw_guest >= 0 && pw_active();
        bool ok;
        if (precision == 2 && !variant_has_f16(v)) ok = false;
        else if (band) ok = v >= BAND_VARIANT_BASE && v < BAND_VARIANT_BASE + BAND_MODES && band_mode_ok(precision, v - BAND_VARIANT_BASE, L);
        else if (v >= PATCH_VARIANT_BASE) ok = v < PATCH_VARIANT_BASE + PATCH_MODES && !hosts_pw && l.out_layer != -2 && L.act <= 1 && L.hout == L.hin &&
                                               conv_patch_supported(L.size, L.stride, L.pad, L.cin, L.cout) && conv_patch_mode_valid(v - PATCH_VARIANT_BASE, L.cin, L.cout);
        else if (v >= PWD_VARIANT_BASE) ok = v < PWD_VARIANT_BASE + PWD_MODES && pwd_candidate(l, L);
        else if (v == BAND_VARIANT_BASE + BANDD_WIDE_MODE) ok = bandd_wide_candidate(l, L);
        else if (v >= RING_VARIANT_BASE) ok = v < RING_VARIANT_BASE + RING_MODES && !hosts_pw && L.act <= 1;
        else ok = v < HV_COUNT && !(hosts_pw && conv_f16s3_variant_info(v).bn < L.cout);
        if (!ok) { set_error("set_tiles: variant %d is not a valid tile of launch %d (layer %d)", v, i, l.layer); return RTOD_E_ARG; }
    }
    tuned[batch] = std::vector<int>(variants, variants + count);
    return RTOD_OK;
}

int Plan::variant_for(const Launch& l, int batch) const {
    const bool band = convs[l.conv_slot].band;
    if (opt_force_f16s3_variant >= 0) {
        const int v = opt_force_f16s3_variant;
        const Layer& FL = layers[l.layer];
        if (band) return band_mode_ok(precision, v - BAND_VARIANT_BASE, FL) ? v : BAND_VARIANT_BASE + band_default_mode(precision, FL);
        if (v == BAND_VARIANT_BASE + BANDD_WIDE_MODE) { if (bandd_wide_candidate(l, FL)) return v; }
        else if (v >= PWD_VARIANT_BASE && v < PWD_VARIANT_BASE + PWD_MODES) { if (pwd_candidate(l, FL)) return v; }
        else if (precision == 1 && v >= RING_VARIANT_BASE && v < RING_VARIANT_BASE + RING_MODES && !(l.pw_guest >= 0 && pw_active()) && FL.act <= 1) return v;
        if (precision == 1 && v >= PATCH_VARIANT_BASE && v < PATCH_VARIANT_BASE + PATCH_MODES && !(l.pw_guest >= 0 && pw_active()) && l.out_layer != -2 && FL.act <= 1 &&
            conv_patch_supported(FL.size, FL.stride, FL.pad, FL.cin, FL.cout) && FL.hout == FL.hin && conv_patch_mode_valid(v - PATCH_VARIANT_BASE, FL.cin, FL.cout)) return v;
        const int g = choose_variant_f16s3(layers[l.layer], batch);
        if (l.pw_guest >= 0 && pw_active() && conv_f16s3_variant_info(g).bn < layers[l.layer].cout) return HV_128x128_8W;
        return g;
    }
    auto it = tuned.find(batch);
    const size_t idx = &l - &launches[0];
    if (it != tuned.end() && idx < it->second.size() && it->second[idx] >= 0) return it->second[idx];
    if (band) return BAND_VARIANT_BASE + band_default_mode(precision, layers[l.layer]);
    const int v = choose_variant_f16s3(layers[l.layer], batch);
    if (l.pw_guest >= 0 && pw_active() && conv_f16s3_variant_info(v).bn < layers[l.layer].cout) return HV_128x128_8W;
    return v;
}

bool Plan::pw_active() const { return precision == 1 && opt_fuse_pointwise; }
bool Plan::bandd_wide_candidate(const Launch& l, const Layer& L) const {
    if (!opt_band_kernel || l.conv_slot < 0 || convs[l.conv_slot].band || !convs[l.conv_slot].split) return false;
    if (l.out_layer == -2 || (l.pw_guest >= 0 && pw_active())) return false;
    const PackedConv& pc = convs[l.conv_slot];
    return conv_bandd_wide_supported(L.size, L.stride, L.pad, pc.cin_p, L.win) && L.hout == L.hin && L.wout == L.win && pc.Npad % 128 == 0 && pc.K == pc.Kpad;
}
bool Plan::pwd_candidate(const Launch& l, const Layer& L) const {
    if (!opt_pwd_kernel || l.conv_slot < 0 || convs[l.conv_slot].band || !convs[l.conv_slot].split) return false;
    if (l.out_layer == -2 || (l.pw_guest >= 0 && pw_active())) return false;
    return conv_pwd_supported(L.size, L.stride, L.pad, convs[l.conv_slot].cin_p) && L.hout == L.hin && L.wout == L.win;
}
bool Plan::stem2_active() const { return precision == 1 && opt_stem2_kernel && stem2_pattern && !keep_all && convs[launches[0].conv_slot].split; }

int Plan::choose_variant_f16s3(const Layer& L, int batch) const {
    if (opt_force_f16s3_variant >= 0 && opt_force_f16s3_variant < HV_COUNT) return opt_force_f16s3_variant;
    if (L.cout <= 64) return HV_128x64;
    const int64_t M = (int64_t)batch * L.hout * L.wout;
    const int64_t gn = (L.cout + 127) / 128;
    if (((M + 127) / 128) * gn >= 512) return HV_128x128;
    if (((M + 63) / 64) * gn >= 512) return HV_64x128;
    return HV_64x64;
}

int Plan::forward(const float* x, int batch, float* out, hipStream_t s, float* launch_ms, bool tune) {
    if (!weights_loaded) { set_error("forward: load_weights has not been called"); return RTOD_E_STATE; }
    if (!x || !out) { set_error("forward: null pointer"); return RTOD_E_ARG; }
    if (batch < 1 || batch > max_batch) { set_error("forward: batch %d outside 1..%d", batch, max_batch); return RTOD_E_ARG; }
    RTOD_HIP(hipSetDevice(device));
    const bool tune_now = tune && precision >= 1 && opt_force_f16s3_variant < 0;
    if (tune_now) { tuning.assign(launches.size(), -1); tune_cache.clear(); }
    const size_t nl = launches.size();
    if (launch_ms && events.size() < 2 * nl) {
        while (events.size() < 2 * nl) { hipEvent_t e; RTOD_HIP(hipEventCreate(&e)); events.push_back(e); }
    }
    for (size_t li = 0; li < nl; ++li) {
        const Launch& l = launches[li];
        if (launch_ms) RTOD_HIP(hipEventRecord(events[2 * li], s));
        int rc = RTOD_OK;
        switch (l.kind) {
            case LK_PACK: {
                View v = view_of(-1);
                rc = launch_pack_input(x, batch, 3, height, width, v.base, 4, s);
                break;
            }
            case LK_CONV: {
                const Layer& L = layers[l.layer];
                const PackedConv& pc = convs[l.conv_slot];
                if (l.pw_host >= 0 && pw_active()) break;
                ConvArgs a;
                rc = build_conv_args(l, batch, out, a);
                if (rc) return rc;
                if (!pc.split) {
                    const int v = choose_variant(L, batch);
                    const int mode = f32_slice_mode(l, batch, v);
                    a.slice_chunks = mode ? pc.slice_chunks : 0;
                    if (mode == 2) { a.partial = d_scratch; a.partial_floats = scratch_floats; }
                    if (opt_bn_batch_stats && L.bn) {
                        if (a.dec.enabled || a.out_split || !d_bn_stats || pc.stats_off < 0) { set_error("forward: layer %d: batch-statistics BatchNorm on an unsupported launch", l.layer); return RTOD_E_STATE; }
                        a.leaky = 0; a.res = nullptr;
                        rc = launch_conv(a, v, s);
                        if (rc) return rc;
                        const View o = view_of(l.out_layer);
                        View r; if (l.in2_layer >= 0) r = view_of(l.in2_layer);
                        rc = launch_bn_batch(o, o, l.in2_layer >= 0 ? &r : nullptr, batch, d_bn_stats + pc.stats_off, pc.Npad, d_weights + pc.bn_off, pc.Npad, L.act, d_bn_partial, bn_partial_count, s);
                    } else
                    rc = launch_conv(a, v, s);
                }
                else if (li == 1 && stem2_active()) {
                    const PackedConv& p0 = convs[launches[0].conv_slot];
                    if (!(l.pw_guest >= 0 && pw_active())) { a.pw_wh = nullptr; a.pw_wl = nullptr; }
                    rc = launch_conv_stem2_f16s3(x, batch, height, width, reinterpret_cast<const _Float16*>(d_weights + p0.w_off),
                                                 reinterpret_cast<const _Float16*>(d_weights + p0.wl_off), d_weights + p0.s_off, d_weights + p0.b_off,
                                                 layers[0].act, a, s);
                } else {
                    if (tune_now) { rc = tune_launch(li, a, batch, s); if (rc) return rc; }
                    rc = launch_split_variant(a, pc, tune_now && tuning[li] >= 0 ? tuning[li] : variant_for(l, batch), s);
                }
                break;
            }
            case LK_STEM: {
                if (stem2_active()) break;
                const Layer& L = layers[l.layer];
                const PackedConv& pc = convs[l.conv_slot];
                const View o = view_of(l.out_layer);
                if (pc.split)
                    rc = launch_conv_stem_split(x, reinterpret_cast<const _Float16*>(d_weights + pc.w_off), reinterpret_cast<const _Float16*>(d_weights + pc.wl_off),
                                                d_weights + pc.s_off, d_weights + pc.b_off, o, batch, height, width, L.hout, L.wout,
                                                L.stride, L.cout, L.act, overflow_flag, s);
                else
                    rc = launch_conv_stem(x, d_weights + pc.w_off, d_weights + pc.b_off, o, batch, height, width, L.hout, L.wout,
                                          L.stride, L.cout, L.act, s);
                break;
            }
            case LK_UPSAMPLE:
                rc = layers[l.layer].nearest ? launch_upsample_nearest2x(view_of(l.in_layer), view_of(l.out_layer), batch, s)
                                             : launch_upsample2x(view_of(l.in_layer), view_of(l.out_layer), batch, s);
                break;
            case LK_MAXPOOL: rc = launch_maxpool(view_of(l.in_layer), view_of(l.out_layer), batch, layers[l.layer].size, layers[l.layer].stride, layers[l.layer].pool_pad, s); break;
            case LK_ADD: rc = launch_add(view_of(l.in_layer), view_of(l.in2_layer), view_of(l.out_layer), batch, s); break;
            case LK_COPY: {
                const View in = view_of(l.in_layer);
                View o; const Buffer& b = bufs[l.out_buf];
                o.base = d_arena + b.offset; o.ldc = b.C; o.coff = l.out_coff; o.C = in.C; o.H = in.H; o.W = in.W;
                rc = launch_copy(in, o, batch, s);
                break;
            }
            case LK_DECODE: {
                const View in = view_of(l.in_layer);
                DecodeArgs d = l.dec; d.train = train_decode;
                rc = launch_decode(in.base + in.coff, (int64_t)in.H * in.W * in.ldc, 1, (int64_t)in.W * in.ldc, in.ldc, batch, d, out, s);
                break;
            }
        }
        if (rc) return rc;
        if (launch_ms) RTOD_HIP(hipEventRecord(events[2 * li + 1], s));
    }
    if (tune_now) tuned[batch] = tuning;
    if (launch_ms) {
        RTOD_HIP(hipEventSynchronize(events[2 * nl - 1]));
        for (size_t li = 0; li < nl; ++li) RTOD_HIP(hipEventElapsedTime(&launch_ms[li], events[2 * li], events[2 * li + 1]));
    }
    return RTOD_OK;
}

void Plan::fill_launch_info(int idx, rtod_launch_info* o, int batch) const {
    memset(o, 0, sizeof(*o));
    const Launch& l = launches[idx];
    o->layer = l.layer; o->kind = l.kind; o->variant = -1;
    if (l.kind == LK_PACK) { o->bytes_per_frame = (int64_t)height * width * (3 + 4) * 4; return; }
    const Layer& L = layers[l.layer];
    o->ksize = L.size; o->stride = L.stride; o->cin = L.cin; o->cout = L.cout; o->hout = L.hout; o->wout = L.wout;
    const int64_t in_b = (int64_t)L.hin * L.win * L.cin * 4, out_b = (int64_t)L.hout * L.wout * L.cout * 4;
    switch (l.kind) {
        case LK_STEM:
            if (stem2_active()) { o->bytes_per_frame = 0; break; }
            o->flops_per_frame = 2ll * L.hout * L.wout * L.cout * L.cin * L.size * L.size;
            o->bytes_per_frame = in_b + out_b;
            o->weight_bytes = ((int64_t)L.cout * L.cin * L.size * L.size + L.cout) * 4;
            break;
        case LK_CONV:
            if (l.pw_host >= 0 && pw_active()) { o->bytes_per_frame = 0; break; }
            if (convs[l.conv_slot].split) o->variant = 100 + variant_for(l, batch);
            else { const int v = choose_variant(L, batch); o->variant = v + 10 * f32_slice_mode(l, batch, v); }
            o->flops_per_frame = 2ll * L.hout * L.wout * L.cout * L.cin * L.size * L.size;
            o->fused_residual = l.in2_layer >= 0; o->fused_decode = l.out_layer == -2;
            o->bytes_per_frame = in_b + out_b + (l.in2_layer >= 0 ? out_b : 0);
            o->weight_bytes = ((int64_t)L.cout * L.cin * L.size * L.size + L.cout) * 4;
            if (idx == 1 && stem2_active()) {
                const Layer& S = layers[0];
                o->variant = 100 + STEM2_VARIANT;
                o->flops_per_frame += 2ll * S.hout * S.wout * S.cout * S.cin * S.size * S.size;
                o->bytes_per_frame = (int64_t)S.hin * S.win * S.cin * 4 + out_b;
                o->weight_bytes += ((int64_t)S.cout * S.cin * S.size * S.size + S.cout) * 4;
            }
            if (l.pw_guest >= 0 && pw_active()) {
                const Layer& G = layers[launches[l.pw_guest].layer];
                o->fused_pointwise = 1;
                o->flops_per_frame += 2ll * G.hout * G.wout * G.cout * G.cin;
                o->bytes_per_frame += (int64_t)G.hout * G.wout * G.cout * 4;
                o->weight_bytes += ((int64_t)G.cout * G.cin + G.cout) * 4;
            }
            break;
        case LK_ADD: o->bytes_per_frame = 3 * out_b; break;
        default: o->bytes_per_frame = in_b + out_b; break;
    }
}

std::string Plan::describe() const {
    std::ostringstream os;
    os << "{\"height\":" << height << ",\"width\":" << width << ",\"total_rows\":" << total_rows << ",\"attrs\":" << attrs
       << ",\"n_weight_floats\":" << n_weight_floats << ",\"conv_flops\":" << conv_flops << ",\"arena_floats\":" << arena_floats
       << ",\"n_launches\":" << launches.size() << ",\"layers\":[";
    for (size_t i = 0; i < layers.size(); ++i) {
        const Layer& L = layers[i];
        if (i) os << ",";
        os << "{\"index\":" << L.index << ",\"type\":\"" << layer_type_name(L.type) << "\",\"cin\":" << L.cin << ",\"cout\":" << L.cout
           << ",\"hin\":" << L.hin << ",\"win\":" << L.win << ",\"hout\":" << L.hout << ",\"wout\":" << L.wout << ",\"size\":" << L.size
           << ",\"stride\":" << L.stride << ",\"pad\":" << L.pad << ",\"bn\":" << (L.bn ? "true" : "false") << ",\"leaky\":" << (L.leaky ? "true" : "false") << ",\"act\":" << L.act << ",\"decode_v5\":" << (L.decode_v5 ? "true" : "false") << ",\"nearest\":" << (L.nearest ? "true" : "false") << ",\"pool_pad\":" << L.pool_pad
           << ",\"srcs\":[";
        for (size_t s = 0; s < L.srcs.size(); ++s) os << (s ? "," : "") << L.srcs[s];
        os << "],\"anchors\":[";
        for (size_t a = 0; a < L.anchors.size(); ++a) os << (a ? "," : "") << "[" << L.anchors[a].first << "," << L.anchors[a].second << "]";
        os << "],\"classes\":" << L.classes << ",\"row_offset\":" << L.row_offset << ",\"rows\":" << L.rows << ",\"w_off\":" << L.w_off
           << ",\"fused_into\":" << ((i == 0 && stem2_active()) ? 1 : L.fused_into) << ",\"fused_away\":" << (L.fused_away ? "true" : "false") << ",\"alias_of\":" << L.alias_of
           << ",\"buf\":" << L.buf << ",\"coff\":" << L.coff << "}";
    }
    os << "],\"bufs\":[";
    for (size_t i = 0; i < bufs.size(); ++i) {
        const Buffer& b = bufs[i];
        if (i) os << ",";
        os << "{\"C\":" << b.C << ",\"H\":" << b.H << ",\"W\":" << b.W << ",\"first\":" << b.first << ",\"last\":" << b.last << ",\"offset\":" << b.offset
           << ",\"floats_per_frame\":" << b.floats_per_frame << "}";
    }
    os << "]}";
    return os.str();
}

}
```

### realtimeobjectdetection_amd/csrc/plan.h

```cpp
#pragma once
#include <map>
#include <string>
#include <vector>

#include "rtod_internal.h"

namespace rtod {

enum LayerType { LT_CONV = 0, LT_SHORTCUT, LT_ROUTE, LT_UPSAMPLE, LT_MAXPOOL, LT_YOLO };
const char* layer_type_name(int t);

struct Layer {
    int index = 0;
    int type = LT_CONV;
    int cin = 0, cout = 0, hin = 0, win = 0, hout = 0, wout = 0;
    int size = 0, stride = 1, pad = 0;
    bool bn = false, leaky = false;
    int act = 0;
    bool nearest = false;
    bool decode_v5 = false;
    int pool_pad = 0;
    std::vector<int> srcs;
    std::vector<std::pair<int, int>> anchors;
    int classes = 0, row_offset = 0, rows = 0;
    int64_t w_off = 0;
    int fused_into = -1;
    bool fused_away = false;
    int buf = -1, coff = 0;
    int alias_of = -1;
};

struct Buffer {
    int C = 0, H = 0, W = 0;
    int first = 0, last = 0;
    int64_t floats_per_frame = 0;
    int64_t offset = 0;
};

enum LaunchKind { LK_CONV = 0, LK_PACK = 1, LK_UPSAMPLE = 2, LK_ADD = 3, LK_MAXPOOL = 4, LK_DECODE = 5, LK_COPY = 6, LK_STEM = 7 };

struct Launch {
    int kind = LK_CONV;
    int layer = 0;
    int in_layer = -1;
    int in2_layer = -1;
    int out_layer = -1;
    int out_buf = -1, out_coff = 0;
    int conv_slot = -1;
    DecodeArgs dec;
    int pw_guest = -1, pw_host = -1;
};

struct PackedConv {
    int layer = 0;
    int cin_p = 0, K = 0, Kpad = 0, Npad = 0;
    int64_t w_off = 0, b_off = 0;
    bool stem = false;
    bool split = false;
    bool band = false;
    int64_t wl_off = 0, s_off = 0;
    int64_t stats_off = -1;
    int64_t bn_off = 0;
    int slice_chunks = 0;
};

struct Plan {
    int height = 0, width = 0, max_batch = 0, device = 0;
    std::map<std::string, std::string> net_info;
    std::vector<Layer> layers;
    std::vector<Buffer> bufs;
    int input_buf = -1;
    std::vector<Launch> launches;
    std::vector<PackedConv> convs;
    int total_rows = 0, attrs = 0;
    int64_t n_weight_floats = 0, conv_flops = 0;
    int64_t arena_floats = 0, packed_floats = 0;
    float* d_arena = nullptr;
    float* d_weights = nullptr;
    double* d_bn_stats = nullptr;
    int64_t bn_stats_doubles = 0;
    double* d_bn_partial = nullptr;
    int64_t bn_partial_count = 0;
    float* d_scratch = nullptr;
    int64_t scratch_floats = 0;
    bool weights_loaded = false;
    int train_decode = 0;
    int precision = 0;
    bool keep_all = false;
    bool opt_fuse_pointwise = true;
    bool opt_stem_kernel = true;
    bool opt_band_kernel = true;
    bool opt_bn_batch_stats = false;
    bool opt_k_slices = true;
    bool opt_k_slice_workgroups = true;
    bool opt_stem2_kernel = true;
    bool opt_patch_kernel = true;
    bool opt_ring_kernel = true;
    bool opt_pwd_kernel = true;
    bool opt_fuse_shortcut = true;
    bool opt_fuse_decode = true;
    bool opt_zero_copy_concat = true;
    int opt_force_f16s3_variant = -1;
    int opt_force_f32_variant = -1;
    int32_t* overflow_flag = nullptr;
    std::vector<hipEvent_t> events;

    ~Plan();
    int parse(const std::string& cfg_text);
    int resolve_shapes();
    int plan_buffers();
    void assign_arena();
    void layout_weights();
    bool uses_split(const Layer& L, int cin_p) const;
    int check_split_supported(int mode) const;
    int load_weights(const float* w, size_t n);
    int forward(const float* x, int batch, float* out, hipStream_t s, float* launch_ms, bool tune = false);
    int set_option(const char* name, int value);
    int set_tiles(int batch, const int* variants, int count);
    void reset_planning();
    View view_of(int layer) const;
    int choose_variant(const Layer& L, int batch) const;
    int choose_variant_f16s3(const Layer& L, int batch) const;
    int build_conv_args(const Launch& l, int batch, float* out, ConvArgs& a) const;
    int tune_launch(size_t li, ConvArgs& a, int batch, hipStream_t s);
    std::vector<int> tuning;
    std::map<std::vector<int>, int> tune_cache;
    int launch_split_variant(ConvArgs& a, const PackedConv& pc, int v, hipStream_t s) const;
    int variant_for(const Launch& l, int batch) const;
    int f32_slice_mode(const Launch& l, int batch, int variant) const;
    bool pw_active() const;
    bool pwd_candidate(const Launch& l, const Layer& L) const;
    bool bandd_wide_candidate(const Launch& l, const Layer& L) const;
    bool stem2_pattern = false;
    bool stem2_active() const;
    std::map<int, std::vector<int>> tuned;
    std::string describe() const;
    void fill_launch_info(int idx, rtod_launch_info* o, int batch) const;
};

}
```

### realtimeobjectdetection_amd/csrc/rtod_internal.h

```cpp
#pragma once
#include <hip/hip_runtime.h>
#if defined(RTOD_STAMPS) && !defined(RTOD_DIAG)
#define RTOD_DIAG 1
#endif
#include <algorithm>
#include <atomic>
#include <cstdint>
#include <cstdio>
#include <string>
#include <vector>

#include "../../include/rtod.h"

namespace rtod {

void set_error(const char* fmt, ...);
int hip_fail(hipError_t e, const char* what);

#define RTOD_HIP(expr)                                              \
    do {                                                            \
        hipError_t _e = (expr);                                     \
        if (_e != hipSuccess) return ::rtod::hip_fail(_e, #expr);   \
    } while (0)

template <typename... Kernel>
int lds_opt_in(std::atomic<unsigned long long>& done, int bytes, const char* who, Kernel... kernels) {
    int dev = 0;
    if (hipGetDevice(&dev) != hipSuccess) return hip_fail(hipGetLastError(), (std::string(who) + " hipGetDevice").c_str());
    if ((done.load(std::memory_order_acquire) >> (dev & 63)) & 1ull) return RTOD_OK;
    for (const void* k : {reinterpret_cast<const void*>(kernels)...})
        if (hipFuncSetAttribute(k, hipFuncAttributeMaxDynamicSharedMemorySize, bytes) != hipSuccess)
            return hip_fail(hipGetLastError(), (std::string(who) + " LDS attribute").c_str());
    done.fetch_or(1ull << (dev & 63), std::memory_order_release);
    return RTOD_OK;
}

inline int device_cu_count() {
    int dev = 0, cus = 0;
    if (hipGetDevice(&dev) != hipSuccess || hipDeviceGetAttribute(&cus, hipDeviceAttributeMultiprocessorCount, dev) != hipSuccess) return 0;
    return cus;
}

struct View {
    int split = 0;
    float* base = nullptr;
    int64_t ldc = 0;
    int coff = 0;
    int C = 0, H = 0, W = 0;
};

struct DecodeArgs {
    int enabled = 0;
    int GH = 0, GW = 0;
    int attrs = 0;
    int n_anchors = 0;
    int train = 0;
    int v5 = 0;
    float stride = 0.f;
    float aw[4] = {0, 0, 0, 0};
    float ah[4] = {0, 0, 0, 0};
    int64_t img_stride = 0;
    int64_t head_off = 0;
};

struct ConvArgs {
    const float* in = nullptr;  int64_t in_ldc = 0;  int in_coff = 0;
    int B = 0, Hi = 0, Wi = 0, Cin = 0;
    const float* w = nullptr;
    const float* bias = nullptr;
    int K = 0, Kpad = 0;
    int Npad = 0;
    int kh = 1, kw = 1, stride = 1, pad = 0;
    int Ho = 0, Wo = 0, Cout = 0;
    float* out = nullptr;       int64_t out_ldc = 0; int out_coff = 0;
    const float* res = nullptr; int64_t res_ldc = 0; int res_coff = 0;
    int leaky = 0;
    DecodeArgs dec;
    const _Float16* w_hi = nullptr;
    const _Float16* w_lo = nullptr;
    const float* inv_scale = nullptr;
    unsigned in_bytes = 0, w_bytes = 0;
    int dbg = 0;
    int32_t* ovf = nullptr;
    int xcd_by_n = 0;
    int out_split = 0;
    int f16 = 0;
    int slice_chunks = 0;
    float* partial = nullptr;
    int64_t partial_floats = 0;
    const _Float16* pw_wh = nullptr;
    const _Float16* pw_wl = nullptr;
    const float* pw_inv_scale = nullptr;
    const float* pw_bias = nullptr;
    float* pw_out = nullptr;    int64_t pw_out_ldc = 0; int pw_out_coff = 0;
    int pw_npad = 0;
    int pw_cout = 0, pw_k = 0, pw_leaky = 0;
};

constexpr float SPLIT_SCALE = 8.0f;
constexpr float ACT_SCALE_F16S3 = SPLIT_SCALE;
constexpr float F16_MAX = 65504.0f;

#ifdef __HIPCC__
__device__ __forceinline__ void split_f16(float v, _Float16& h, _Float16& l, float& amax) {
    amax = fmaxf(amax, fabsf(v));
    const float vc = __builtin_amdgcn_fmed3f(v, -F16_MAX, F16_MAX);
    h = (_Float16)vc;
    l = (_Float16)(vc - (float)h);
}
__device__ __forceinline__ _Float16 f16_sat(float v, float& amax) {
    amax = fmaxf(amax, fabsf(v));
    return (_Float16)__builtin_amdgcn_fmed3f(v, -F16_MAX, F16_MAX);
}
__device__ __forceinline__ float apply_act(float v, int act) {
    if (act == 1) return v > 0.f ? v : v * 0.1f;
    if (act == 2) return v / (1.0f + expf(-v));
    return v;
}
__device__ __forceinline__ void split_overflow_report(int32_t* flag, float amax) {
    if (flag && !(amax <= F16_MAX)) atomicOr(flag, 1);
}
__device__ __forceinline__ __amdgpu_buffer_rsrc_t buffer_rsrc(const void* p, unsigned bytes) {
    return __builtin_amdgcn_make_buffer_rsrc(const_cast<void*>(p), 0, bytes, 0x00020000);
}
__device__ __forceinline__ int xcd_remap(int id, int n) {
    const int q = n >> 3, r = n & 7, xcd = id & 7;
    return (xcd < r ? xcd * (q + 1) : r * (q + 1) + (xcd - r) * q) + (id >> 3);
}
#endif

constexpr int EPI_F16 = 8;

enum ConvVariant { CV_128x128 = 0, CV_128x64 = 1, CV_64x64 = 2, CV_128x32 = 3, CV_COUNT };
struct ConvVariantInfo { int bm, bn; const char* name; };
const ConvVariantInfo& conv_variant_info(int v);
int conv_f32_kernel_name(int variant, char* buf, size_t len);
int launch_conv(const ConvArgs& a, int variant, hipStream_t s);
int conv_f32_slices(const ConvArgs& a);
enum ConvF16Variant { HV_128x128 = 0, HV_128x64 = 1, HV_64x64 = 2, HV_64x128 = 3, HV_256x128 = 4, HV_128x256 = 5, HV_128x128_8W = 6, HV_128x64_8W = 7, HV_256x128_16W = 8,
                      HV_192x128_8W = 9, HV_96x128_8W = 10, HV_192x128_12W = 11, HV_COUNT };
const ConvVariantInfo& conv_f16s3_variant_info(int v);
int conv_f16s3_kernel_name(int variant, int epi, char* buf, size_t len);
int launch_conv_f16s3(const ConvArgs& a, int variant, hipStream_t s);
bool conv_band_supported(int ksize, int stride, int pad, int cin, int w_in);
constexpr int BANDD_MODES = 9;
constexpr int BAND_LDS_MODES = 11;
constexpr int BAND_MODES = BAND_LDS_MODES + BANDD_MODES;
static_assert(50 + BAND_MODES <= 70, "band variant ids end where the ring kernel's begin");
constexpr int BAND_K2_MODE0 = 7;
const ConvVariantInfo& conv_bandd_mode_info(int idx);
int conv_bandd_mode_kg(int idx);
constexpr int BANDD_WIDE_MODE = BAND_LDS_MODES + 7;
bool conv_bandd_wide_supported(int ksize, int stride, int pad, int cin, int w_in);
int conv_bandd_kernel_name(int idx, int epi, char* buf, size_t len);
int launch_conv_bandd_f16s3(const ConvArgs& a, int idx, hipStream_t s);
int conv_band_layer_kg(int cin, int h, int w);
bool conv_band_mode_valid(int mode, int cin, int h, int w);
int conv_band_default_mode(int cin, int h, int w);
const ConvVariantInfo& conv_band_mode_info(int mode);
int conv_band_kernel_name(int mode, int epi, char* buf, size_t len);
int launch_conv_band_f16s3(const ConvArgs& a, int mode, hipStream_t s);
constexpr int BAND_VARIANT_BASE = 50;
constexpr int RING_MODES = 8;
constexpr int RING_VARIANT_BASE = 70;
const ConvVariantInfo& conv_ring_mode_info(int mode);
int conv_ring_kernel_name(int mode, int epi, char* buf, size_t len);
int launch_conv_ring_f16s3(const ConvArgs& a, int mode, hipStream_t s);
constexpr int PWD_MODES = 11;
constexpr int PWD_VARIANT_BASE = 90;
bool conv_pwd_supported(int ksize, int stride, int pad, int cin);
const ConvVariantInfo& conv_pwd_mode_info(int mode);
int conv_pwd_kernel_name(int mode, int epi, char* buf, size_t len);
int launch_conv_pwd_f16s3(const ConvArgs& a, int mode, hipStream_t s);
constexpr int STEM2_VARIANT = 130;
bool conv_stem2_supported(int k0, int s0, int p0, int cin0, int cout0, int k1, int s1, int p1, int cout1, int pw_cout);
int conv_stem2_kernel_name(int pw, char* buf, size_t len);
int launch_conv_stem2_f16s3(const float* x, int B, int H, int W, const _Float16* w0h, const _Float16* w0l, const float* inv0, const float* bias0,
                            int leaky0, const ConvArgs& c1, hipStream_t s);
constexpr int PATCH_MODES = 5;
constexpr int PATCH_WRES_MODE = 4;
bool conv_patch_mode_valid(int mode, int cin, int cout);
constexpr int PATCH_VARIANT_BASE = 110;
bool conv_patch_supported(int ksize, int stride, int pad, int cin, int cout);
const ConvVariantInfo& conv_patch_mode_info(int mode);
int conv_patch_kernel_name(int mode, int epi, char* buf, size_t len);
int launch_conv_patch_f16s3(const ConvArgs& a, int mode, hipStream_t s);

int launch_conv_stem(const float* x_nchw, const float* w, const float* bias, const View& out, int B, int H, int W,
                     int Ho, int Wo, int stride, int Cout, int leaky, hipStream_t s);
int launch_conv_stem_split(const float* x_nchw, const _Float16* wh, const _Float16* wl, const float* inv_scale, const float* bias,
                           const View& out, int B, int H, int W, int Ho, int Wo, int stride, int Cout, int leaky, int32_t* ovf, hipStream_t s);
int launch_prep_image(const unsigned char* img, int h, int w, int bgr, int inp_dim, float* out, hipStream_t s);
int launch_prep_frames(const unsigned char* frames, int batch, int h, int w, int bgr, int out_h, int out_w, float* out, hipStream_t s);
int launch_pack_input(const float* x_nchw, int B, int C, int H, int W, float* out_nhwc, int Cp, hipStream_t s);
int launch_upsample2x(const View& in, const View& out, int B, hipStream_t s);
int launch_add(const View& a, const View& b, const View& out, int B, hipStream_t s);
int launch_maxpool(const View& in, const View& out, int B, int size, int stride, int pad, hipStream_t s);
int launch_upsample_nearest2x(const View& in, const View& out, int B, hipStream_t s);
int launch_bn_batch(const View& x, const View& y, const View* res, int B, double* stats, int sstride, const float* bn, int gstride, int act,
                    double* partial, int64_t partial_doubles, hipStream_t s);
size_t bn_partial_doubles(int max_channels);
struct BnUpdateEntry { float* running_mean; float* running_var; int64_t stats_off; double unbias; int sstride; int channels; };
constexpr int BN_UPDATE_MAX = 32;
struct BnUpdateTable { BnUpdateEntry e[BN_UPDATE_MAX]; };
int launch_bn_update_running(const BnUpdateEntry* entries, int n, const double* stats, double momentum, hipStream_t s);
int launch_copy(const View& in, const View& out, int B, hipStream_t s);
int launch_view_to_nchw(const View& in, int B, float* out_nchw, hipStream_t s);
int launch_decode(const float* raw, int64_t sb, int64_t sc, int64_t sy, int64_t sx, int B,
                  const DecodeArgs& d, float* out, hipStream_t s);
int launch_confidence_mask(const float* pred, int64_t rows, int attrs, float conf, float* out, hipStream_t s);
int launch_bbox_iou(const float* box1, const float* boxes, int k, int row_stride, float* iou, hipStream_t s);

size_t nms_workspace_bytes(int batch, int n);
int launch_write_results(const float* pred, int batch, int n, int num_class, float conf, float nms,
                         float* out, int cap, int32_t* counts, void* ws, size_t ws_bytes, hipStream_t s);
int launch_nms_class_offset(const float* pred, int batch, int n, int num_class, float conf, float iou_thr, float max_wh, int max_det,
                            float* out, int cap, int32_t* counts, void* ws, size_t ws_bytes, hipStream_t s);

}
```

Baseline: 2530 frames/s.

## Add 2D patch-tiled direct 3x3 conv kernel and fused decode in pwd epilogue

Adds a new direct-convolution kernel (patchd) for 3x3 stride-1/2 layers. Each workgroup DMA-loads a spatial input patch (TH rows by 16 columns plus halo) into double-buffered LDS and reuses it across all nine taps, feeding split-f16 MFMA. It also generalises the shared band epilogue to non-linear pixel mappings and to a fused YOLO decode pass, which lets the pointwise kernel take detection-head layers. The autotuner gains the new variants as candidates, so it can pick them only where they measure faster. The cost is more code paths and more tuning time.

Result: no change. 2551 frames/s (median of 6 runs) (+0.8%).

```diff
diff --git a/realtimeobjectdetection_amd/csrc/capi.cpp b/realtimeobjectdetection_amd/csrc/capi.cpp
--- a/realtimeobjectdetection_amd/csrc/capi.cpp
+++ b/realtimeobjectdetection_amd/csrc/capi.cpp
@@ -105,6 +105,7 @@
 
 const char* rtod_conv_variant_name(int variant) {
     if (variant == 100 + STEM2_VARIANT) return "conv_stem2_f16s3<2 x 4x16, stem + 3x3 s2 + 1x1>";
+    if (variant >= 100 + PATCHD_VARIANT_BASE && variant < 100 + PATCHD_VARIANT_BASE + PATCHD_MODES) return conv_patchd_mode_info(variant - 100 - PATCHD_VARIANT_BASE).name;
     if (variant >= 100 + PATCH_VARIANT_BASE && variant < 100 + PATCH_VARIANT_BASE + PATCH_MODES) return conv_patch_mode_info(variant - 100 - PATCH_VARIANT_BASE).name;
     if (variant >= 100 + PWD_VARIANT_BASE && variant < 100 + PWD_VARIANT_BASE + PWD_MODES) return conv_pwd_mode_info(variant - 100 - PWD_VARIANT_BASE).name;
     if (variant >= 100 + RING_VARIANT_BASE && variant < 100 + RING_VARIANT_BASE + RING_MODES) return conv_ring_mode_info(variant - 100 - RING_VARIANT_BASE).name;
@@ -121,7 +122,8 @@
 int rtod_conv_kernel_name(int variant, int epilogue, char* buf, size_t len) {
     if (!buf || len == 0) { set_error("conv_kernel_name: null buffer"); return RTOD_E_ARG; }
     int n = -1;
-    if (variant >= 100 + PATCH_VARIANT_BASE) n = conv_patch_kernel_name(variant - 100 - PATCH_VARIANT_BASE, epilogue, buf, len);
+    if (variant >= 100 + PATCHD_VARIANT_BASE) n = conv_patchd_kernel_name(variant - 100 - PATCHD_VARIANT_BASE, epilogue, buf, len);
+    else if (variant >= 100 + PATCH_VARIANT_BASE) n = conv_patch_kernel_name(variant - 100 - PATCH_VARIANT_BASE, epilogue, buf, len);
     else if (variant >= 100 + PWD_VARIANT_BASE) n = conv_pwd_kernel_name(variant - 100 - PWD_VARIANT_BASE, epilogue, buf, len);
     else if (variant >= 100 + RING_VARIANT_BASE) n = conv_ring_kernel_name(variant - 100 - RING_VARIANT_BASE, epilogue, buf, len);
     else if (variant >= 100 + BAND_VARIANT_BASE) n = conv_band_kernel_name(variant - 100 - BAND_VARIANT_BASE, epilogue, buf, len);
diff --git a/realtimeobjectdetection_amd/csrc/conv_bandd_common.h b/realtimeobjectdetection_amd/csrc/conv_bandd_common.h
--- a/realtimeobjectdetection_amd/csrc/conv_bandd_common.h
+++ b/realtimeobjectdetection_amd/csrc/conv_bandd_common.h
@@ -22,9 +22,13 @@
     else vmcnt<NBASE + 5 * PER>();
 }
 
-template <int BM, int BN, int WM, int WN, int NT, int RG, bool RES, int KG, bool F16 = false>
+struct BanddLinearRows {};
+template <int BM, int BN, int WM, int WN, int NT, int RG, bool RES, int KG, bool F16 = false, class PIX = BanddLinearRows, bool DEC = false>
 __device__ __forceinline__ void bandd_epilogue(const ConvArgs& a, f32x4 (&acc)[WM / 16][WN / 16], unsigned char* smem, int bm, int bn, int tid,
-                                               int wm, int wn, int lr, int lh, int M, int kg) {
+                                               int wm, int wn, int lr, int lh, int M, int kg, const PIX& pix = PIX()) {
+    constexpr bool LINEAR = std::is_same<PIX, BanddLinearRows>::value;
+    static_assert(!DEC || (!RES && KG == 1 && LINEAR), "decode pass: plain linear tiles");
+    static_assert(!DEC || NT % BN == 0 || BN % NT == 0, "decode mapping");
     constexpr int TM = WM / 16, TN = WN / 16, MT = 16, NE = 4, TS = BN;
     static_assert(BM % RG == 0 && RG % 16 == 0, "epilogue pass");
 #ifdef RTOD_TIMELINE
@@ -33,7 +37,7 @@
 #endif
     float* T = reinterpret_cast<float*>(smem);
     float amax = 0.f;
-    const float escale = SPLIT_SCALE;
+    const float escale = DEC ? 1.0f : SPLIT_SCALE;
     constexpr int GPR = BN / 8;
     constexpr int NG = (RG * GPR + NT - 1) / NT;
     constexpr int NP = BM / RG;
@@ -61,6 +65,10 @@
             for (int i = 0; i < NG; ++i) {
                 const int m = bm * BM + p * RG + er + i * RSTEP;
                 const _Float16* qq = (er + i * RSTEP < RG && m < M && ecol) ? q : rh0;
+                if constexpr (!LINEAR) {
+                    const int r = p * RG + er + i * RSTEP;
+                    qq = (er + i * RSTEP < RG && pix.ok(r) && ecol) ? rh0 + (int64_t)pix.pixel(r) * 2 * a.res_ldc + ec8 : rh0;
+                }
                 rq_h[p][i] = *reinterpret_cast<const f16x8*>(qq);
                 if constexpr (!F16) rq_l[p][i] = *reinterpret_cast<const f16x8*>(qq + a.res_ldc);
                 q += rstep;
@@ -117,13 +125,66 @@
         BD_ESTAMP(1)
         __syncthreads();
         BD_ESTAMP(2)
+        if constexpr (DEC) {
+            constexpr int DSTEP = NT / BN > 0 ? NT / BN : 1;
+            const int hw = a.Ho * a.Wo;
+            for (int nl = tid % BN; nl < BN; nl += NT) {
+                const int n = bn * BN + nl;
+                if (n >= a.Cout) continue;
+                const int an = n / a.dec.attrs, c = n - an * a.dec.attrs;
+                const bool is_wh = (c == 2 || c == 3) && !a.dec.train;
+                const bool is_raw = (c == 2 || c == 3) && a.dec.train;
+                const float anc = (c == 2 ? a.dec.aw[an] : a.dec.ah[an]);
+                const int r0 = (NT >= BN) ? tid / BN : 0;
+                int m = bm * BM + rg + r0;
+                const int b = m / hw;
+                int cell = m - b * hw;
+                int gy = cell / a.dec.GW, gx = cell - gy * a.dec.GW;
+                float* op = a.out + (int64_t)b * a.dec.img_stride + a.dec.head_off + (int64_t)cell * a.Cout + n;
+                const int64_t row_step = (int64_t)DSTEP * a.Cout;
+                const int64_t img_fix = a.dec.img_stride - (int64_t)hw * a.Cout;
+                if (a.dec.v5) {
+                    for (int r = r0; r < RG && m < M; r += DSTEP, m += DSTEP) {
+                        const float sg = __builtin_amdgcn_rcpf(1.0f + __expf(-T[r * TS + nl]));
+                        float o = sg;
+                        if (c < 2) o = ((sg * 2.0f - 0.5f) + (float)(c == 0 ? gx : gy)) * a.dec.stride;
+                        else if (c < 4) { const float t2 = sg * 2.0f; o = (t2 * t2) * anc; }
+                        *op = o;
+                        op += row_step; cell += DSTEP; gx += DSTEP;
+                        while (gx >= a.dec.GW) { gx -= a.dec.GW; ++gy; }
+                        while (cell >= hw) { cell -= hw; gy -= a.dec.GH; op += img_fix; }
+                    }
+                } else
+                for (int r = r0; r < RG && m < M; r += DSTEP, m += DSTEP) {
+                    const float v = T[r * TS + nl];
+                    float o;
+                    if (is_raw) o = v;
+                    else {
+                        const float ex = __expf(is_wh ? v : -v);
+                        if (is_wh) o = (ex * anc) * a.dec.stride;
+                        else {
+                            o = __builtin_amdgcn_rcpf(1.0f + ex);
+                            if (c < 2 && !a.dec.train) o = (o + (float)(c == 0 ? gx : gy)) * a.dec.stride;
+                        }
+                    }
+                    *op = o;
+                    op += row_step; cell += DSTEP; gx += DSTEP;
+                    while (gx >= a.dec.GW) { gx -= a.dec.GW; ++gy; }
+                    while (cell >= hw) { cell -= hw; gy -= a.dec.GH; op += img_fix; }
+                }
+            }
+        } else {
         _Float16* oq = reinterpret_cast<_Float16*>(a.out) + a.out_coff + bn * BN + (int64_t)(bm * BM + rg + er) * 2 * a.out_ldc + ec8;
         const int64_t ostep = (int64_t)RSTEP * 2 * a.out_ldc;
 #pragma unroll
         for (int gi = 0; gi < NG; ++gi, oq += ostep) {
             const int r = er + gi * RSTEP;
             const int m = bm * BM + rg + r;
-            if (r >= RG || m >= M || !ecol) continue;
+            if constexpr (LINEAR) { if (r >= RG || m >= M || !ecol) continue; }
+            else {
+                if (r >= RG || !pix.ok(rg + r) || !ecol) continue;
+                oq = reinterpret_cast<_Float16*>(a.out) + a.out_coff + bn * BN + (int64_t)pix.pixel(rg + r) * 2 * a.out_ldc + ec8;
+            }
             const f32x4 v0 = *reinterpret_cast<const f32x4*>(T + r * TS + ec8);
             const f32x4 v1 = *reinterpret_cast<const f32x4*>(T + r * TS + ec8 + 4);
             float v[8] = {v0[0], v0[1], v0[2], v0[3], v1[0], v1[1], v1[2], v1[3]};
@@ -148,6 +209,7 @@
                 store_act16(oq, ph, false);
                 store_act16(oq + a.out_ldc, pl, false);
             }
+        }
         }
         BD_ESTAMP(3)
         if (rg + RG < BM) __syncthreads();
@@ -156,7 +218,7 @@
 #ifdef RTOD_TIMELINE
     if (threadIdx.x == 0 && blockIdx.x < BD_EPI_BLOCKS) for (int i = 0; i < 5; ++i) g_bandd_epi[blockIdx.x * 5 + i] = et_[i];
 #endif
-    split_overflow_report(a.ovf, amax);
+    if constexpr (!DEC) split_overflow_report(a.ovf, amax);
 }
 
 }
diff --git a/realtimeobjectdetection_amd/csrc/conv_patchd_f16s3.hip b/realtimeobjectdetection_amd/csrc/conv_patchd_f16s3.hip
--- /dev/null
+++ b/realtimeobjectdetection_amd/csrc/conv_patchd_f16s3.hip
@@ -0,0 +1,241 @@
+#include "conv_bandd_common.h"
+#include <cstdio>
+
+namespace rtod {
+
+constexpr int PD_BN = 128, PD_NW = 4, PD_TW = 16;
+
+__host__ __device__ constexpr int patchd_rows(int th, int s) { return s == 1 ? (th + 2) * 18 : (2 * th + 1) * 33; }
+__host__ __device__ constexpr int patchd_blocks(int th, int s) { return ((patchd_rows(th, s) + 15) / 16 + PD_NW - 1) / PD_NW * PD_NW; }
+__host__ __device__ constexpr int patchd_rg(int bm) { return bm * PD_BN * 4 <= 32768 ? bm : (bm / 2) * PD_BN * 4 <= 32768 ? bm / 2 : bm / 4; }
+
+struct PatchdRows {
+    int H, W, y0, x0, m00;
+    __device__ __forceinline__ bool ok(int r) const { return y0 + (r >> 4) < H && x0 + (r & 15) < W; }
+    __device__ __forceinline__ int pixel(int r) const { return m00 + (r >> 4) * W + (r & 15); }
+};
+
+template <int TH, int S, int BUFM, int MINW, int EPI>
+__global__ __launch_bounds__(PD_NW * 64, MINW)
+void conv_patchd_f16s3_kernel(const ConvArgs a, const int tiles_x, const int tiles_y, const int grid_n) {
+    static_assert(S == 1 || S == 2, "stride");
+    static_assert(EPI == EPI_SPLIT || EPI == EPI_SPLIT_RES, "patchd epilogues");
+    constexpr bool DB = BUFM == 1;
+    constexpr int BM = TH * 16, BN = PD_BN, NW = PD_NW, NT = NW * 64, WN = BN / NW;
+    constexpr int TM = TH, TN = WN / 16;
+    constexpr int NB = 2 * TN;
+    constexpr int UNITS = 9 * TM;
+    constexpr int PC = S == 1 ? 18 : 33;
+    constexpr int PE = patchd_rows(TH, S);
+    constexpr int NBLKP = patchd_blocks(TH, S), PPW = NBLKP / NW;
+    constexpr int PLANE = NBLKP * 1024, BUF = 2 * PLANE;
+    constexpr int RG = patchd_rg(BM);
+    static_assert(PPW <= 5 || !DB, "bandd_wait_vmcnt_plus covers 5 pairs");
+    static_assert(((TH - 1) * S + 2) * PC + (S == 1 ? 2 : 17) + 15 < PE, "the last unit reads inside the patch");
+
+    extern __shared__ __attribute__((aligned(16))) unsigned char smem[];
+    const int W = a.Wi, H = a.Hi;
+    const int tid = (int)threadIdx.x;
+    const int wave = __builtin_amdgcn_readfirstlane(tid >> 6), lane = tid & 63;
+    const int lr = lane & 15, lh = lane >> 4;
+
+    const int nwg = a.B * tiles_y * tiles_x * grid_n;
+    int u = xcd_remap((int)blockIdx.x, nwg);
+    const int bn = u % grid_n; u /= grid_n;
+    const int x0 = (u % tiles_x) * PD_TW; u /= tiles_x;
+    const int y0 = (u % tiles_y) * TH;
+    const int tb = u / tiles_y;
+    const int iy0 = y0 * S - 1, ix0 = x0 * S - 1;
+    const unsigned PS = (unsigned)a.in_ldc * 4u;
+    const unsigned lo_plane = (unsigned)a.in_ldc * 2u;
+
+    const __amdgpu_buffer_rsrc_t rs_a = buffer_rsrc(a.in, a.in_bytes);
+    const __amdgpu_buffer_rsrc_t rs_wh = buffer_rsrc(a.w_hi, a.w_bytes);
+    const __amdgpu_buffer_rsrc_t rs_wl = buffer_rsrc(a.w_lo, a.w_bytes);
+    const unsigned lds0 = (unsigned)(size_t)smem;
+
+    auto dma_patch = [&](int cc, int buf) __attribute__((always_inline)) {
+        const unsigned soff = (unsigned)cc * 64u;
+        const unsigned base = lds0 + (unsigned)(buf * BUF);
+        int l = (int)threadIdx.x;
+        asm volatile("" : "+v"(l));
+        const int lrow = (l & 63) >> 2;
+        const unsigned cpart = (unsigned)(a.in_coff + ((l & 3) ^ ((lrow >> 1) & 3)) * 8) * 2u;
+#pragma unroll
+        for (int k = 0; k < PPW; ++k) {
+            const int blk = wave + k * NW;
+            const int q = blk * 16 + lrow;
+            const int py = q / PC, rem = q - py * PC;
+            const int px = S == 1 ? rem : (rem < 17 ? 2 * rem : 2 * rem - 33);
+            const int iy = iy0 + py, ix = ix0 + px;
+            const bool ok = q < PE && (unsigned)iy < (unsigned)H && (unsigned)ix < (unsigned)W;
+            const unsigned vo = ok ? (unsigned)((tb * H + iy) * W + ix) * PS + cpart : OOB;
+            const unsigned dst = base + (unsigned)blk * 1024u;
+            lds_dma_pair(rs_a, rs_a, vo, soff, lo_plane + soff, dst, dst + PLANE);
+        }
+    };
+    const int n0 = bn * BN + wave * WN;
+    const unsigned bvoff = n0 + lr < a.Npad ? (unsigned)((n0 + lr) * 32 + lh * 8) * 2u : OOB;
+    const unsigned wchunk = (unsigned)a.Npad * (HBK * 2);
+    const int n_cc = a.Cin / 32;
+    const int nsteps = 9 * n_cc;
+    u32x4 Bq[3][TN][2];
+    int ld_step = 0, ld_cc = 0, ld_tap = 0;
+    auto load_b = [&](u32x4 (&q)[TN][2]) __attribute__((always_inline)) {
+        const unsigned vo = ld_step < nsteps ? bvoff : OOB;
+        const unsigned koff = (unsigned)(ld_cc * 9 + ld_tap) * wchunk;
+        q[0][0] = buffer_load_b128(rs_wh, vo, koff);
+        q[0][1] = buffer_load_b128(rs_wl, vo, koff);
+        q[1][0] = buffer_load_b128<1024>(rs_wh, vo, koff);
+        q[1][1] = buffer_load_b128<1024>(rs_wl, vo, koff);
+        ++ld_step;
+        if (++ld_tap == 9) { ld_tap = 0; ++ld_cc; }
+    };
+
+    f32x4 acc[TM][TN];
+#pragma unroll
+    for (int i = 0; i < TM; ++i)
+#pragma unroll
+        for (int j = 0; j < TN; ++j)
+#pragma unroll
+            for (int e = 0; e < 4; ++e) acc[i][j][e] = 0.f;
+
+    const int lh4 = lh << 4;
+    f16x8 Ah[3], Al[3];
+    typedef const f16x8 __attribute__((address_space(3))) lds_f16x8;
+    int lr_c = lr;
+    int abase[8];
+    auto read_unit = [&](int t, int i, f16x8& h, f16x8& l) __attribute__((always_inline)) {
+        const int ky = t / 3, kx = t % 3;
+        const int c = S == 1 ? (i + ky) * PC + kx : (2 * i + ky) * PC + (kx & 1) * 17 + (kx >> 1);
+        const int o = abase[c & 7] + c * 64;
+        h = *reinterpret_cast<lds_f16x8*>((unsigned)o);
+        l = *reinterpret_cast<lds_f16x8*>((unsigned)(o + PLANE));
+    };
+
+    dma_patch(0, 0);
+    load_b(Bq[0]);
+    load_b(Bq[1]);
+    if constexpr (DB) {
+        vmcnt<0>();
+        tie_bset<false>(Bq[0]); tie_bset<false>(Bq[1]);
+        __builtin_amdgcn_sched_barrier(0);
+    }
+    __builtin_amdgcn_s_setprio(2);
+#pragma unroll 1
+    for (int cc = 0; cc < n_cc; ++cc) {
+        const int buf = DB ? (cc & 1) : 0;
+        const int bufoff = (int)lds0 + buf * BUF;
+        asm volatile("" : "+v"(lr_c));
+#pragma unroll
+        for (int m = 0; m < 8; ++m) abase[m] = bufoff + (lr_c << 6) + ((((lr_c + m) << 3) ^ lh4) & 0x30);
+        if constexpr (!DB) {
+            if (cc > 0) {
+                __builtin_amdgcn_s_barrier();
+                dma_patch(cc, 0);
+            }
+            vmcnt<0>();
+            tie_bset<false>(Bq[0]); tie_bset<false>(Bq[1]);
+        }
+        int dma_behind = 0;
+        __builtin_amdgcn_sched_barrier(0);
+        __builtin_amdgcn_s_barrier();
+        if constexpr (DB) { if (cc + 1 < n_cc) { dma_patch(cc + 1, buf ^ 1); dma_behind = PPW; } }
+        read_unit(0, 0, Ah[0], Al[0]);
+        read_unit(1 / TM, 1 % TM, Ah[1], Al[1]);
+        __builtin_amdgcn_sched_barrier(0);
+#pragma unroll
+        for (int un = 0; un < UNITS; ++un) {
+            const int t = un / TM, i = un % TM;
+            if (i == 0) {
+                load_b(Bq[(t + 2) % 3]);
+                if constexpr (DB) {
+                    if (t >= 2) vmcnt<2 * NB>(); else bandd_wait_vmcnt_plus<2 * NB, 2>(dma_behind);
+                    tie_bset<false>(Bq[t % 3]);
+                } else if (t >= 2) { vmcnt<2 * NB>(); tie_bset<false>(Bq[t % 3]); }
+                __builtin_amdgcn_sched_barrier(0);
+            }
+            if (un + 2 < UNITS) read_unit((un + 2) / TM, (un + 2) % TM, Ah[(un + 2) % 3], Al[(un + 2) % 3]);
+            const f16x8 ah = Ah[un % 3], al = Al[un % 3];
+#pragma unroll
+            for (int j = 0; j < TN; ++j) {
+                const f16x8 bh = __builtin_bit_cast(f16x8, Bq[t % 3][j][0]);
+                const f16x8 bl = __builtin_bit_cast(f16x8, Bq[t % 3][j][1]);
+                acc[i][j] = __builtin_amdgcn_mfma_f32_16x16x32_f16(al, bh, acc[i][j], 0, 0, 0);
+                acc[i][j] = __builtin_amdgcn_mfma_f32_16x16x32_f16(ah, bl, acc[i][j], 0, 0, 0);
+                acc[i][j] = __builtin_amdgcn_mfma_f32_16x16x32_f16(ah, bh, acc[i][j], 0, 0, 0);
+            }
+            __builtin_amdgcn_sched_barrier(0);
+        }
+    }
+    vmcnt<0>();
+    tie_bset<false>(Bq[0]); tie_bset<false>(Bq[1]); tie_bset<false>(Bq[2]);
+    __builtin_amdgcn_sched_barrier(0);
+    __builtin_amdgcn_s_setprio(0);
+
+    const PatchdRows rows{a.Ho, a.Wo, y0, x0, (tb * a.Ho + y0) * a.Wo + x0};
+    bandd_epilogue<BM, BN, BM, WN, NT, RG, EPI == EPI_SPLIT_RES, 1, false>(a, acc, smem, 0, bn, tid, 0, wave, lr, lh, a.B * a.Ho * a.Wo, 0, rows);
+}
+
+template <int TH, int S, int BUFM, int MINW>
+static int launch_patchd(const ConvArgs& a, hipStream_t s) {
+    constexpr int BM = TH * 16, NT = PD_NW * 64;
+    const int tiles_x = (a.Wo + PD_TW - 1) / PD_TW, tiles_y = (a.Ho + TH - 1) / TH, gn = (a.Cout + PD_BN - 1) / PD_BN;
+    const int64_t wgs = (int64_t)a.B * tiles_x * tiles_y * gn;
+    if (wgs >= (1ll << 30)) { set_error("launch_conv_patchd: too many tiles"); return RTOD_E_ARG; }
+    constexpr int main_bytes = (BUFM == 1 ? 2 : 1) * patchd_blocks(TH, S) * 2048;
+    constexpr int epi_bytes = patchd_rg(BM) * PD_BN * 4;
+    constexpr int lds = main_bytes > epi_bytes ? main_bytes : epi_bytes;
+    static_assert(lds <= 160 * 1024, "LDS budget");
+    auto k_res = conv_patchd_f16s3_kernel<TH, S, BUFM, MINW, EPI_SPLIT_RES>;
+    auto k_plain = conv_patchd_f16s3_kernel<TH, S, BUFM, MINW, EPI_SPLIT>;
+    static std::atomic<unsigned long long> attr_done{0};
+    if (int rc = lds_opt_in(attr_done, lds, "conv_patchd_f16s3", k_res, k_plain)) return rc;
+    if (a.res) hipLaunchKernelGGL(k_res, dim3((unsigned)wgs), dim3(NT), lds, s, a, tiles_x, tiles_y, gn);
+    else hipLaunchKernelGGL(k_plain, dim3((unsigned)wgs), dim3(NT), lds, s, a, tiles_x, tiles_y, gn);
+    return hip_fail(hipGetLastError(), "conv_patchd_f16s3 launch");
+}
+
+#define RTOD_PATCHD_TILES(X) \
+    X(0, 8, 1, 1, 3, ",db") X(1, 4, 2, 0, 3, "") X(2, 8, 2, 0, 2, "")
+
+#define RTOD_X_INFO(mode, th, st, db, minw, sfx) {th * 16, PD_BN, "conv_patchd_f16s3<" #th "x16x128,s" #st sfx ">"},
+static const ConvVariantInfo kPatchdModes[PATCHD_MODES] = { RTOD_PATCHD_TILES(RTOD_X_INFO) };
+#undef RTOD_X_INFO
+const ConvVariantInfo& conv_patchd_mode_info(int mode) { return kPatchdModes[mode < 0 || mode >= PATCHD_MODES ? 0 : mode]; }
+int conv_patchd_mode_stride(int mode) {
+#define RTOD_X_STRIDE(m, th, st, db, minw, sfx) if (mode == m) return st;
+    RTOD_PATCHD_TILES(RTOD_X_STRIDE)
+#undef RTOD_X_STRIDE
+    return 0;
+}
+bool conv_patchd_supported(int ksize, int stride, int pad, int cin) {
+    return ksize == 3 && (stride == 1 || stride == 2) && pad == 1 && cin % 32 == 0;
+}
+int conv_patchd_kernel_name(int mode, int epi, char* buf, size_t len) {
+#define RTOD_X_NAME(m, th, st, db, minw, sfx) \
+    if (mode == m) return snprintf(buf, len, "void rtod::conv_patchd_f16s3_kernel<" #th ", " #st ", " #db ", " #minw ", %d>(rtod::ConvArgs, int, int, int)", epi);
+    RTOD_PATCHD_TILES(RTOD_X_NAME)
+#undef RTOD_X_NAME
+    return -1;
+}
+
+int launch_conv_patchd_f16s3(const ConvArgs& a, int mode, hipStream_t s) {
+    if (int rc = check_split_conv_args(a, "launch_conv_patchd", false)) return rc;
+    if (!conv_patchd_supported(a.kh, a.stride, a.pad, a.Cin) || a.kw != 3 || a.Ho != (a.Hi - 1) / a.stride + 1 || a.Wo != (a.Wi - 1) / a.stride + 1 ||
+        a.dec.enabled || a.pw_wh || a.f16) {
+        set_error("launch_conv_patchd: unsupported layer (k=%d s=%d pad=%d Cin=%d)", a.kh, a.stride, a.pad, a.Cin); return RTOD_E_ARG;
+    }
+    if (a.in_ldc % 8 || a.in_coff % 8 || a.out_ldc % 8 || a.out_coff % 8 || a.Cout % 8 || a.K != a.Kpad || a.K != 9 * a.Cin || a.Npad % 128) {
+        set_error("launch_conv_patchd: bad view / K"); return RTOD_E_ARG;
+    }
+    switch (mode) {
+#define RTOD_X_CASE(m, th, st, db, minw, sfx) case m: if (a.stride != st) break; return launch_patchd<th, st, db, minw>(a, s);
+        RTOD_PATCHD_TILES(RTOD_X_CASE)
+#undef RTOD_X_CASE
+    }
+    set_error("launch_conv_patchd: mode %d unsupported (stride %d)", mode, a.stride);
+    return RTOD_E_ARG;
+}
+
+}
diff --git a/realtimeobjectdetection_amd/csrc/conv_pwd_f16s3.hip b/realtimeobjectdetection_amd/csrc/conv_pwd_f16s3.hip
--- a/realtimeobjectdetection_amd/csrc/conv_pwd_f16s3.hip
+++ b/realtimeobjectdetection_amd/csrc/conv_pwd_f16s3.hip
@@ -141,7 +141,9 @@
     __builtin_amdgcn_sched_barrier(0);
     __builtin_amdgcn_s_setprio(0);
 
-    bandd_epilogue<BM, BN, BM, 32, NT, RG, epi_kind(EPI) == EPI_SPLIT_RES, 1, F16>(a, acc, smem, bm, bn, tid, 0, wn, lr, lh, M, 0);
+    static_assert(epi_kind(EPI) == EPI_SPLIT || epi_kind(EPI) == EPI_SPLIT_RES || EPI == EPI_DECODE, "slab tile epilogues");
+    if constexpr (EPI == EPI_DECODE) bandd_epilogue<BM, BN, BM, 32, NT, RG, false, 1, false, BanddLinearRows, true>(a, acc, smem, bm, bn, tid, 0, wn, lr, lh, M, 0);
+    else bandd_epilogue<BM, BN, BM, 32, NT, RG, epi_kind(EPI) == EPI_SPLIT_RES, 1, F16>(a, acc, smem, bm, bn, tid, 0, wn, lr, lh, M, 0);
 }
 
 template <int BM, int NW, int NST, int MINW>
@@ -158,11 +160,13 @@
     const int fe = a.f16 ? 1 : 0;
     auto k_res = fe ? conv_pwd_f16s3_kernel<BM, NW, NST, MINW, EPI_SPLIT_RES | EPI_F16> : conv_pwd_f16s3_kernel<BM, NW, NST, MINW, EPI_SPLIT_RES>;
     auto k_plain = fe ? conv_pwd_f16s3_kernel<BM, NW, NST, MINW, EPI_SPLIT | EPI_F16> : conv_pwd_f16s3_kernel<BM, NW, NST, MINW, EPI_SPLIT>;
+    auto k_dec = conv_pwd_f16s3_kernel<BM, NW, NST, MINW, EPI_DECODE>;
     if constexpr (lds > 64 * 1024) {
         static std::atomic<unsigned long long> attr_done[2] = {{0}, {0}};
-        if (int rc = lds_opt_in(attr_done[fe], lds, "conv_pwd_f16s3", k_res, k_plain)) return rc;
-    }
-    if (a.res) hipLaunchKernelGGL(k_res, dim3(gm * gn), dim3(NT), lds, s, ax, gm, gn);
+        if (int rc = lds_opt_in(attr_done[fe], lds, "conv_pwd_f16s3", k_res, k_plain, k_dec)) return rc;
+    }
+    if (a.dec.enabled) hipLaunchKernelGGL(k_dec, dim3(gm * gn), dim3(NT), lds, s, ax, gm, gn);
+    else if (a.res) hipLaunchKernelGGL(k_res, dim3(gm * gn), dim3(NT), lds, s, ax, gm, gn);
     else hipLaunchKernelGGL(k_plain, dim3(gm * gn), dim3(NT), lds, s, ax, gm, gn);
     return hip_fail(hipGetLastError(), "conv_pwd_f16s3 launch");
 }
@@ -187,7 +191,7 @@
 
 int launch_conv_pwd_f16s3(const ConvArgs& a, int idx, hipStream_t s) {
     if (int rc = check_split_conv_args(a, "launch_conv_pwd", true)) return rc;
-    if (!conv_pwd_supported(a.kh, a.stride, a.pad, a.Cin) || a.kw != 1 || a.Ho != a.Hi || a.Wo != a.Wi || a.dec.enabled || a.pw_wh) {
+    if (!conv_pwd_supported(a.kh, a.stride, a.pad, a.Cin) || a.kw != 1 || a.Ho != a.Hi || a.Wo != a.Wi || (a.dec.enabled && (a.f16 || a.res)) || a.pw_wh) {
         set_error("launch_conv_pwd: unsupported shape (k=%d s=%d pad=%d Cin=%d)", a.kh, a.stride, a.pad, a.Cin); return RTOD_E_ARG;
     }
     if (a.in_ldc % 8 || a.in_coff % 8 || a.K != a.Kpad || a.K != a.Cin || a.Npad % 128) { set_error("launch_conv_pwd: bad view / K"); return RTOD_E_ARG; }
diff --git a/realtimeobjectdetection_amd/csrc/plan.cpp b/realtimeobjectdetection_amd/csrc/plan.cpp
--- a/realtimeobjectdetection_amd/csrc/plan.cpp
+++ b/realtimeobjectdetection_amd/csrc/plan.cpp
@@ -304,6 +304,7 @@
     }
     else if (k == "k_slice_workgroups") flag = &opt_k_slice_workgroups;
     else if (k == "patch_kernel") flag = &opt_patch_kernel;
+    else if (k == "patchd_kernel") flag = &opt_patchd_kernel;
     else if (k == "stem_kernel") flag = &opt_stem_kernel;
     else if (k == "band_kernel") flag = &opt_band_kernel;
     else if (k == "fuse_shortcut") flag = &opt_fuse_shortcut;
@@ -788,6 +789,10 @@
 
 int Plan::launch_split_variant(ConvArgs& a, const PackedConv& pc, int v, hipStream_t s) const {
     if (precision == 2 && !variant_has_f16(v)) { set_error("variant %d has no plain-f16 instance", v); return RTOD_E_STATE; }
+    if (v >= PATCHD_VARIANT_BASE) {
+        if (pc.band) { set_error("patch variant requested for a band layer"); return RTOD_E_STATE; }
+        return launch_conv_patchd_f16s3(a, v - PATCHD_VARIANT_BASE, s);
+    }
     if (v >= PATCH_VARIANT_BASE) {
         if (pc.band) { set_error("patch variant requested for a band layer"); return RTOD_E_STATE; }
         return launch_conv_patch_f16s3(a, v - PATCH_VARIANT_BASE, s);
@@ -862,7 +867,7 @@
     const bool pw = a.pw_wh != nullptr;
     const std::vector<int> key = {L.cin, L.cout, L.size, L.stride, L.hout, L.wout, l.in2_layer >= 0, l.out_layer == -2, pw ? a.pw_cout : 0,
                                   convs[l.conv_slot].band ? 1 : 0, opt_ring_kernel ? 1 : 0, opt_patch_kernel ? 1 : 0, opt_pwd_kernel ? 1 : 0, L.act,
-                                  precision, L.hin, L.win, L.pad};
+                                  precision, L.hin, L.win, L.pad, opt_patchd_kernel ? 1 : 0};
     auto it = tune_cache.find(key);
     if (it != tune_cache.end()) { tuning[li] = it->second; return RTOD_OK; }
     std::vector<int> gkey = key; gkey.push_back(device); gkey.push_back(batch);
@@ -890,6 +895,7 @@
                 cand.push_back(PATCH_VARIANT_BASE + m);
             }
         if (bandd_wide_candidate(l, L)) cand.push_back(BAND_VARIANT_BASE + BANDD_WIDE_MODE);
+        for (int m = 0; m < PATCHD_MODES; ++m) if (patchd_candidate(l, L, m)) cand.push_back(PATCHD_VARIANT_BASE + m);
         if (pwd_candidate(l, L))
             for (int m = 0; m < PWD_MODES; ++m) {
                 if (conv_pwd_mode_info(m).bn > 128 && conv_pwd_mode_info(m).bn > (L.cout + 127) / 128 * 128) continue;
@@ -956,6 +962,7 @@
         bool ok;
         if (precision == 2 && !variant_has_f16(v)) ok = false;
         else if (band) ok = v >= BAND_VARIANT_BASE && v < BAND_VARIANT_BASE + BAND_MODES && band_mode_ok(precision, v - BAND_VARIANT_BASE, L);
+        else if (v >= PATCHD_VARIANT_BASE) ok = v < PATCHD_VARIANT_BASE + PATCHD_MODES && patchd_candidate(l, L, v - PATCHD_VARIANT_BASE);
         else if (v >= PATCH_VARIANT_BASE) ok = v < PATCH_VARIANT_BASE + PATCH_MODES && !hosts_pw && l.out_layer != -2 && L.act <= 1 && L.hout == L.hin &&
                                                conv_patch_supported(L.size, L.stride, L.pad, L.cin, L.cout) && conv_patch_mode_valid(v - PATCH_VARIANT_BASE, L.cin, L.cout);
         else if (v >= PWD_VARIANT_BASE) ok = v < PWD_VARIANT_BASE + PWD_MODES && pwd_candidate(l, L);
@@ -975,6 +982,7 @@
         const Layer& FL = layers[l.layer];
         if (band) return band_mode_ok(precision, v - BAND_VARIANT_BASE, FL) ? v : BAND_VARIANT_BASE + band_default_mode(precision, FL);
         if (v == BAND_VARIANT_BASE + BANDD_WIDE_MODE) { if (bandd_wide_candidate(l, FL)) return v; }
+        else if (v >= PATCHD_VARIANT_BASE && v < PATCHD_VARIANT_BASE + PATCHD_MODES) { if (patchd_candidate(l, FL, v - PATCHD_VARIANT_BASE)) return v; }
         else if (v >= PWD_VARIANT_BASE && v < PWD_VARIANT_BASE + PWD_MODES) { if (pwd_candidate(l, FL)) return v; }
         else if (precision == 1 && v >= RING_VARIANT_BASE && v < RING_VARIANT_BASE + RING_MODES && !(l.pw_guest >= 0 && pw_active()) && FL.act <= 1) return v;
         if (precision == 1 && v >= PATCH_VARIANT_BASE && v < PATCH_VARIANT_BASE + PATCH_MODES && !(l.pw_guest >= 0 && pw_active()) && l.out_layer != -2 && FL.act <= 1 &&
@@ -1001,8 +1009,19 @@
 }
 bool Plan::pwd_candidate(const Launch& l, const Layer& L) const {
     if (!opt_pwd_kernel || l.conv_slot < 0 || convs[l.conv_slot].band || !convs[l.conv_slot].split) return false;
+    if ((l.out_layer == -2 && precision != 1) || (l.pw_guest >= 0 && pw_active())) return false;
+    return conv_pwd_supported(L.size, L.stride, L.pad, convs[l.conv_slot].cin_p) && L.hout == L.hin && L.wout == L.win;
+}
+bool Plan::patchd_candidate(const Launch& l, const Layer& L, int mode) const {
+    if (!opt_patchd_kernel || precision != 1 || l.conv_slot < 0 || convs[l.conv_slot].band || !convs[l.conv_slot].split) return false;
     if (l.out_layer == -2 || (l.pw_guest >= 0 && pw_active())) return false;
-    return conv_pwd_supported(L.size, L.stride, L.pad, convs[l.conv_slot].cin_p) && L.hout == L.hin && L.wout == L.win;
+    const PackedConv& pc = convs[l.conv_slot];
+    const int st = conv_patchd_mode_stride(mode);
+    if (!conv_patchd_supported(L.size, L.stride, L.pad, pc.cin_p) || L.stride != st || pc.Npad % 128 || pc.K != pc.Kpad || L.cout % 8) return false;
+    if (L.hout != (L.hin - 1) / st + 1 || L.wout != (L.win - 1) / st + 1) return false;
+    const View in = view_of(l.in_layer), out = view_of(l.out_layer);
+    if (in.ldc % 8 || in.coff % 8 || out.ldc % 8 || out.coff % 8) return false;
+    return L.cout > 64 && (st == 2 || L.win > 94);
 }
 bool Plan::stem2_active() const { return precision == 1 && opt_stem2_kernel && stem2_pattern && !keep_all && convs[launches[0].conv_slot].split; }
 
diff --git a/realtimeobjectdetection_amd/csrc/plan.h b/realtimeobjectdetection_amd/csrc/plan.h
--- a/realtimeobjectdetection_amd/csrc/plan.h
+++ b/realtimeobjectdetection_amd/csrc/plan.h
@@ -97,6 +97,7 @@
     bool opt_patch_kernel = true;
     bool opt_ring_kernel = true;
     bool opt_pwd_kernel = true;
+    bool opt_patchd_kernel = true;
     bool opt_fuse_shortcut = true;
     bool opt_fuse_decode = true;
     bool opt_zero_copy_concat = true;
@@ -130,6 +131,7 @@
     int f32_slice_mode(const Launch& l, int batch, int variant) const;
     bool pw_active() const;
     bool pwd_candidate(const Launch& l, const Layer& L) const;
+    bool patchd_candidate(const Launch& l, const Layer& L, int mode) const;
     bool bandd_wide_candidate(const Launch& l, const Layer& L) const;
     bool stem2_pattern = false;
     bool stem2_active() const;
diff --git a/realtimeobjectdetection_amd/csrc/rtod_internal.h b/realtimeobjectdetection_amd/csrc/rtod_internal.h
--- a/realtimeobjectdetection_amd/csrc/rtod_internal.h
+++ b/realtimeobjectdetection_amd/csrc/rtod_internal.h
@@ -185,6 +185,13 @@
 const ConvVariantInfo& conv_patch_mode_info(int mode);
 int conv_patch_kernel_name(int mode, int epi, char* buf, size_t len);
 int launch_conv_patch_f16s3(const ConvArgs& a, int mode, hipStream_t s);
+constexpr int PATCHD_MODES = 3;
+constexpr int PATCHD_VARIANT_BASE = 140;
+bool conv_patchd_supported(int ksize, int stride, int pad, int cin);
+int conv_patchd_mode_stride(int mode);
+const ConvVariantInfo& conv_patchd_mode_info(int mode);
+int conv_patchd_kernel_name(int mode, int epi, char* buf, size_t len);
+int launch_conv_patchd_f16s3(const ConvArgs& a, int mode, hipStream_t s);
 
 int launch_conv_stem(const float* x_nchw, const float* w, const float* bias, const View& out, int B, int H, int W,
                      int Ho, int Wo, int stride, int Cout, int leaky, hipStream_t s);
```
